# lmb-freiburg/understanding_flow_robustness

Measured on AMD Instinct MI355X. Metric: attack-iters/s, higher is better.
Workload: dtype f32

## Files before the change

include/ufr_hip.h:

```cpp
#ifndef UFR_HIP_H_
#define UFR_HIP_H_

#include <stdint.h>

#ifdef __cplusplus
extern "C" {
#endif

#define UFR_ABI_VERSION 9

enum { UFR_F32 = 0, UFR_F64 = 1, UFR_F16 = 2 };
enum {
  UFR_OK = 0,
  UFR_EINVAL = -1,
  UFR_EUNSUPPORTED = -2,
  UFR_ELAUNCH = -3
};

typedef void* ufr_stream_t;

int ufr_abi_version(void);
const char* ufr_last_error(void);
int ufr_device_count(void);
const char* ufr_build_manifest(void);
// ... 55 lines not shown
  float* grad_vol[UFR_MAX_LEVELS];
  int Hl[UFR_MAX_LEVELS], Wl[UFR_MAX_LEVELS];
} ufr_pyramid;

int ufr_corr_lookup_forward(const ufr_pyramid* pyr, const float* coords, float* out, int B, int H1,
                            int W1, int radius, ufr_stream_t stream);
int ufr_corr_lookup_backward(const ufr_pyramid* pyr, const float* coords, const float* grad_out,
                             int B, int H1, int W1, int radius, ufr_stream_t stream);

int ufr_resample2d_forward(const float* input1, const float* input2, float* output, int B, int C,
                           int Hi, int Wi, int H, int W, int kernel_size, int bilinear,
                           ufr_stream_t stream);
int ufr_resample2d_backward(const float* input1, const float* input2, const float* grad_output,
                            float* grad_input1, float* grad_input2, int B, int C, int Hi, int Wi,
                            int H, int W, int kernel_size, int bilinear, ufr_stream_t stream);
long ufr_resample2d_backward_workspace_bytes(int B, int H, int W);
int ufr_resample2d_backward_owner(const float* input1, const float* input2, const float* grad_output, float* grad_input1,
                                  float* grad_input2, void* workspace, long workspace_bytes, int B, int C, int H, int W,
                                  ufr_stream_t stream);

int ufr_flow_upscale4_forward(const float* flow, float* out, int B, int h, int w, int bilinear, float scale, int divide,
                              ufr_stream_t stream);
int ufr_flow_upscale4_backward(const float* grad_out, float* grad_flow, int B, int h, int w, int bilinear, float scale, int divide,
                               ufr_stream_t stream);
int ufr_fn2_stage_pack(const float* x, const float* resampled, const float* flow, float* out, int B, int H, int W, float div_flow,
                       ufr_stream_t stream);
int ufr_fn2_stage_unpack_grad(const float* grad_out, const float* packed, float* grad_x, float* grad_resampled, int B, int H, int W,
                              ufr_stream_t stream);
int ufr_fn2_stage_finish_grad(const float* grad_out, const float* grad_image, const float* grad_flow_rs, float* grad_x, float* grad_flow,
                              int B, int H, int W, float div_flow, ufr_stream_t stream);
int ufr_fn2_fusion_pack(const float* x, const float* flow_sd, const float* flow_s2, const float* res_sd, const float* res_s2, float* out,
                        int B, int H, int W, ufr_stream_t stream);
int ufr_fn2_fusion_unpack_grad(const float* grad_out, const float* packed, const float* res_sd, const float* res_s2, float* grad_x,
                               float* grad_res_sd, float* grad_res_s2, float* grad_flow_sd, float* grad_flow_s2, int B, int H, int W,
                               ufr_stream_t stream);
int ufr_fn2_fusion_finish_grad(const float* grad_image_sd, const float* grad_image_s2, const float* grad_flow_rs_sd,
                               const float* grad_flow_rs_s2, float* grad_x, float* grad_flow_sd, float* grad_flow_s2, int B, int H, int W,
                               ufr_stream_t stream);

int ufr_channelnorm_forward(const float* input1, float* output, int B, int C, int H, int W,
                            int norm_deg, ufr_stream_t stream);
int ufr_channelnorm_backward(const float* input1, const float* output, const float* grad_output,
                             float* grad_input1, int B, int C, int H, int W, int norm_deg,
                             ufr_stream_t stream);

int ufr_patch_paste(const float* tgt, const float* ref, const float* patch, const float* mask,
                    float* adv_tgt, float* adv_ref, int B, int CHW, long patch_bstride,
                    long mask_bstride, int do_clamp, float lo, float hi, ufr_stream_t stream);
int ufr_patch_update(const float* tgt, const float* ref, const float* g_tgt, const float* g_ref,
                     float* patch, const float* mask, float* adv_tgt, float* adv_ref, int B, int CHW,
                     long patch_bstride, long mask_bstride, float step, float bound, float lo, float hi,
                     const float* gate_state, ufr_stream_t stream);
int ufr_attack_gate(const float* loss_cur, float* state, float threshold, ufr_stream_t stream);
int ufr_patch_grad_crop(const float* g_tgt, const float* g_ref, const float* mask_p, const int* origins,
                        const int* origins_host, const float* loss_local, float* rows, int B, int H, int W,
                        int ph, int pw, int groups, ufr_stream_t stream);
int ufr_patch_grad_crop_window(const float* gxw, const int* win, const float* mask_p, const int* origins, const float* loss_local,
                               float* rows, int B, int H, int W, int wh, int ww, int ph, int pw, int groups, ufr_stream_t stream);
int ufr_patch_apply(const float* rows, int n_rows, float* patch_p, float* loss, int ph, int pw, float step,
                    float bound, const float* gate_state, ufr_stream_t stream);
int ufr_patch_paste_placed(const float* tgt, const float* ref, const float* patch_p, const float* mask_p,
                           const int* origins, const int* origins_host, float* adv_tgt, float* adv_ref,
                           float* mask_out, int B, int H, int W, int ph, int pw, int do_clamp, float lo, float hi,
                           const float* gate_state, ufr_stream_t stream);
int ufr_patch_paste_placed_rect(const float* tgt, const float* ref, const float* patch_p, const float* mask_p,
                                const int* origins, float* adv_tgt, float* adv_ref, int B, int H, int W, int ph, int pw,
                                int do_clamp, float lo, float hi, const float* gate_state, ufr_stream_t stream);
int ufr_attack_load_frames(const float* tgt, const float* ref, const float* patch_p, const float* mask_p, const int* origins,
                           float* tgt_dst, float* ref_dst, float* adv_tgt, float* adv_ref, int B, int H, int W, int ph, int pw,
                           ufr_stream_t stream);
int ufr_patch_mask_placed(const float* mask_p, const int* origins, float* mask_out, int B, int H, int W, int ph, int pw,
                          ufr_stream_t stream);
int ufr_patch_grad_crop_packed(const float* G, const int* win, const float* mask_p, const int* origins, const float* loss_local,
                               float* rows, int B, int H, int W, int wh, int ww, int ph, int pw, int groups, ufr_stream_t stream);
int ufr_patch_apply_paste_rect(const float* rows, int n_rows, float* patch_p, float* loss, const float* tgt, const float* ref,
                               const float* mask_p, const int* origins, float* adv_tgt, float* adv_ref, int B, int H, int W, int ph,
                               int pw, float step, float bound, int do_clamp, float lo, float hi, const float* gate_state,
                               ufr_stream_t stream);
#define UFR_LOSS_PARTIALS 1024
int ufr_flow_loss(const float* flow, const float* target, float* grad_flow, float* loss, int B,
                  int HW, int kind, float weight, float* partials, ufr_stream_t stream);
int ufr_flow2_upsampled_loss(const float* flow2, float flow_scale, const float* target, float* grad_flow2, float* loss, int B,
                             int h, int w, int kind, float weight, float* partials, ufr_stream_t stream);

int ufr_gru_gates_forward(const float* zr_pre, const float* h, float* z_out, float* rh_out, int B, int Ch,
                          int HW, long rh_bstride, ufr_stream_t stream);
int ufr_gru_gates_backward(const float* zr_pre, const float* h, const float* g_z, const float* g_rh,
                           float* g_zr, float* g_h, int B, int Ch, int HW, long grh_bstride,
                           ufr_stream_t stream);
int ufr_gru_blend_forward(const float* q_pre, const float* z, const float* h, float* h_out, long total,
                          ufr_stream_t stream);
int ufr_gru_blend_backward(const float* q_pre, const float* z, const float* h, const float* g, float* g_qpre,
                           float* g_z, float* g_h, long total, ufr_stream_t stream);

int ufr_raft_flow_patches(const float* flow, void* planes, long plane_stride, int chunk0, int B, int H, int W, ufr_stream_t stream);
int ufr_raft_motion_finish(void* p1, long plane_stride1, void* p2, long plane_stride2, int chunk0, const float* flow, int B, int H,
                           int W, ufr_stream_t stream);
int ufr_raft_motion_finish_slabs(const float* ws, int splitk, int Npad, int N, const float* bias, float slope, void* p1, long plane_stride1,
                                 void* p2, long plane_stride2, int chunk0, const float* flow, int B, int H, int W, ufr_stream_t stream);
int ufr_raft_coords_step(float* coords1, const float* delta, const float* coords0, float* saved, float* flow, long n, ufr_stream_t stream);
int ufr_grad_finalize_consume(float* g, const void* mask_plane0, void* out, long out_plane_stride, long M, int chunks, float slope,
                              ufr_stream_t stream);
int ufr_gru_gates_cm_forward(float* zr, const void* h, long h_plane_stride, int h_chunk0, void* rh, long rh_plane_stride,
                             int rh_chunk0, long M, int chunks, ufr_stream_t stream);
int ufr_gru_gates_cm_forward_slabs(const float* ws, int splitk, int Npad, const float* bias, const float* addend, float* zr, const void* h,
                                   long h_plane_stride, int h_chunk0, void* rh, long rh_plane_stride, int rh_chunk0, long M, int chunks,
                                   ufr_stream_t stream);
int ufr_gru_blend_cm_forward_slabs(const float* ws, int splitk, int Npad, const float* bias, const float* addend, float* q, const float* z,
                                   const void* h, long h_plane_stride, int h_chunk0, void* out, long out_plane_stride, int out_chunk0,
                                   long M, int chunks, ufr_stream_t stream);
int ufr_gru_blend_cm_forward(float* q, const float* z, const void* h, long h_plane_stride, int h_chunk0, void* out,
                             long out_plane_stride, int out_chunk0, long M, int chunks, ufr_stream_t stream);
int ufr_gru_blend_cm_backward(const float* q, const float* z, const void* h, long h_plane_stride, int h_chunk0, const float* g,
                              void* gq, long gq_plane_stride, int gq_chunk0, float* g_z, float* g_h, long M, int chunks,
                              float* acc_gq, ufr_stream_t stream);
int ufr_gru_gates_cm_backward(const float* zr, const void* h, long h_plane_stride, int h_chunk0, const float* g_z, float* g_rh,
                              void* gzr, long gzr_plane_stride, int gzr_chunk0, float* g_h, long M, int chunks, int consume_g_rh,
                              float* acc_gzr, ufr_stream_t stream);

long ufr_cm_norm_workspace_doubles(long HW, int n, int chunks);
int ufr_cm_norm_stats(const float* x, float* stats, double* workspace, long HW, int n, int chunks, float eps, ufr_stream_t stream);
int ufr_cm_norm_apply(const float* x, const float* stats, const void* res, long res_plane_stride, int res_chunk0, void* out,
                      long out_plane_stride, int out_chunk0, long HW, int n, int chunks, int relu1, int relu2, ufr_stream_t stream);
int ufr_cm_norm_stats_apply(const float* x, float* stats, double* workspace, float eps, const void* res, long res_plane_stride,
                            int res_chunk0, void* out, long out_plane_stride, int out_chunk0, long HW, int n, int chunks, int relu1,
                            int relu2, ufr_stream_t stream);
int ufr_cm_norm_backward(const float* x, const float* G, const void* outmask, int mask_chunk0, const float* stats, float* sums,
                         double* workspace, void* gz, long gz_plane_stride, int gz_chunk0, long HW, int n, int chunks, int relu1,
                         ufr_stream_t stream);
int ufr_cm_masked_copy(const float* G, const void* outmask, long mask_elem_offset, float* out, long elems, ufr_stream_t stream);

int ufr_conv3x3s2_c3_planes(const float* frames, const float* weight, const float* bias, float slope, void* out_planes,
                            long plane_stride, int out_chunk0, int n, int N, int H, int W, ufr_stream_t stream);

int ufr_conv3x3_c16_planes(const void* in_planes, long in_plane_stride, int in_chunk0, const float* weight_ct16, const float* bias,
                           float slope, void* out_planes, long out_plane_stride, int out_chunk0, int n, int H, int W, ufr_stream_t stream);

int ufr_pwc_warp_forward(const float* x, const float* flow, float* out, int B, int C, int H, int W,
                         ufr_stream_t stream);
int ufr_pwc_warp_backward(const float* x, const float* flow, const float* grad_out, float* grad_x, float* grad_flow,
                          int B, int C, int H, int W, ufr_stream_t stream);
long ufr_pwc_warp_backward_workspace_bytes(int B, int H, int W);
int ufr_pwc_warp_backward_owner(const float* x, const float* flow, const float* grad_out, float* grad_x, float* grad_flow,
                                void* workspace, long workspace_bytes, int B, int C, int H, int W, ufr_stream_t stream);

int ufr_raft_normalize_pair(const float* image1, const float* image2, float* stack, long n_each, ufr_stream_t stream);
int ufr_raft_normalize_pair_backward(const float* grad_stack, float* grad1, float* grad2, long n_each, ufr_stream_t stream);
int ufr_raft_fmap_pyramid_forward(const float* fmap, float* const* levels_nhwc, int levels, int B, int C, int H, int W,
                                  ufr_stream_t stream);
int ufr_raft_fmap_pyramid_backward(const float* const* grad_levels_nhwc, int levels, float* grad_fmap, int B, int C, int H, int W,
                                   ufr_stream_t stream);

int ufr_raft_context_split_forward(const float* ctx, float* net, float* inp, int B, int Ct, int Cr, long HW, ufr_stream_t stream);
int ufr_raft_context_split_backward(const float* net, const float* inp, const float* g_net, const float* g_inp, float* g_ctx,
                                    int B, int Ct, int Cr, long HW, ufr_stream_t stream);

int ufr_convex_upsample_forward(const float* flow, const float* mask, float* up, int N, int H, int W,
                                ufr_stream_t stream);
int ufr_convex_upsample_backward(const float* flow, const float* mask, const float* grad_up, float* grad_flow,
                                 float* grad_mask, float* workspace, int N, int H, int W, ufr_stream_t stream);

int ufr_flow_loss_ex(const float* flow, const float* gt, float* grad_flow, float* loss, int B, int HW,
                     int gt_channels, int kind, float scale, const float* scale_dev, float* partials,
                     ufr_stream_t stream);
int ufr_universal_update(const float* img0, const float* img1, const float* g0, const float* g1,
                         float* grad_sum, float* adv0, float* adv1, float* delta, int B, int CHW,
// ... 95 lines not shown
  int on;
  int row_tiles, col_tiles;
  int full_row_tiles, tail_row_tiles;
  int tail_row0, tail_rows;
  int slices, slice_ktiles, ktiles;
  int workgroups;
  long ws_floats;
  int steps_before, steps_after;
} ufr_igemm_tail_plan_t;
int ufr_igemm_tail_plan(const ufr_igemm_desc* d, int resident_workgroups, ufr_igemm_tail_plan_t* plan);
int ufr_igemm_balanced(const ufr_igemm_desc* d, int resident_workgroups, float* ws, long ws_floats, ufr_stream_t stream);
typedef struct {
  const void* x; long x_plane_stride; int in_chunk0, C;
  const void* gy; long gy_plane_stride; int g_chunk0, N;
  int B, Hi, Wi, Ho, Wo, kh, kw, sy, sx, py, px;
  float* dw;
  float* db;
  int accumulate;
  int splitm; float* ws; long ws_elems;
  int products;
} ufr_igemm_wgrad_desc;
int ufr_igemm_wgrad(const ufr_igemm_wgrad_desc* d, ufr_stream_t stream);
int ufr_igemm_wgrad_dilated(const ufr_igemm_wgrad_desc* d, int dy, int dx, ufr_stream_t stream);
int ufr_igemm_variant_fallbacks(void);
int ufr_igemm_clock_probe(unsigned long long* buf, int capacity_workgroups);
int ufr_rowmajor_to_planes(const float* src, long ld, long rows, int cols, float scale, void* planes, long plane_stride, int chunk0,
                           long plane_rows, ufr_stream_t stream);
int ufr_nchw_to_planes(const float* x, void* planes, long plane_stride, int chunk0, int B, int C, int H, int W,
                       float scale, float slope, const float* bias, ufr_stream_t stream);
int ufr_window_scatter_planes(const float* src, void* planes, long plane_stride, int chunk0, const int* win, int n_win,
                              int N, int C, int Hd, int Wd, int wh, int ww, int level_stride, int margin,
                              ufr_stream_t stream);
int ufr_window_features_planes(const void* c2w, long c2w_stride, const void* c3w, long c3w_stride, void* cat2, long cat2_stride,
                               void* c3a, long c3a_stride, void* c3b, long c3b_stride, float* c3_nchw, float* c3w_nchw,
                               const int* win, int B, int H, int W, int wh, int ww, int m2, int m3, ufr_stream_t stream);
int ufr_chunks_to_nchw(const void* planes, long plane_stride, const float* f32, int chunk0, const void* mask,
                       int mask_chunk0, float* out, int B, int C, int H, int W, float scale, float slope,
                       ufr_stream_t stream);
int ufr_nchw_cat_to_planes(const float* const* srcs, const int* channels, const int* dst_channel0, int nseg, void* planes,
                           long plane_stride, int chunk0, int chunks, int B, int H, int W, ufr_stream_t stream);
int ufr_chunks_to_nchw_cat(const float* g, int chunk0, int chunks, float* const* dsts, const int* channels, const int* src_channel0,
                           int nseg, const float* act0, float pos0, float neg0, int B, int H, int W, ufr_stream_t stream);
int ufr_grad_finalize(const float* g, int g_chunk0, const void* mask, int mask_chunk0, void* out, long out_plane_stride,
                      int out_chunk0, long M, int chunks, float slope, ufr_stream_t stream);

int ufr_conv1_direct(const float* frames_a, const float* frames_b, int Ba, int Bb, int H, int W, const double* mean,
                     const void* wimg, const float* bias, float slope, void* out_planes, long plane_stride, int out_chunk0,
                     ufr_stream_t stream);
int ufr_conv1_pack_planes(const float* frames_a, const float* frames_b, void* planes, long plane_stride, int Ba, int Bb, int H,
                          int W, const double* mean, ufr_stream_t stream);
int ufr_conv1_unpack_grad(const float* G, float* grad_frames, int N, int H, int W, ufr_stream_t stream);
int ufr_unshuffle_pack_planes(const float* x, void* planes, long plane_stride, int N, int C, int H, int W, ufr_stream_t stream);
int ufr_unshuffle_unpack_grad(const float* G, float* grad_x, int N, int C, int H, int W, ufr_stream_t stream);
int ufr_nchw_grad_to_planes(const float* grad, const float* act, void* planes, long plane_stride, int chunk0, int B, int C, int H,
                            int W, float slope, ufr_stream_t stream);
int ufr_window_gather_chunks(const float* src, float* dst, const int* win, int n_win, int N, int N_dst, int chunks, int Hs, int Ws,
                             int wh, int ww, int level_stride, int margin, ufr_stream_t stream);

int ufr_normalize_frames(const float* frames_a, const float* frames_b, float* out, int Ba, int Bb, int C, int H, int W,
                         const double* mean, ufr_stream_t stream);

int ufr_corr_forward_planes_window(const void* f1_planes, const void* f2_planes, long in_plane_stride, void* out_planes,
                                   long out_plane_stride, int out_chunk0, int B, int C, int H, int W, int patch,
                                   int dilation_patch, float scale, float slope, const int* win, int level_stride,
                                   int win_cells, ufr_stream_t stream);

int ufr_corr_forward_planes_changed(const void* f1_planes, const void* f2_planes, long in_plane_stride, void* out_planes,
                                    long out_plane_stride, int out_chunk0, int B, int C, int H, int W, int patch,
                                    int dilation_patch, float scale, float slope, const int* win, int level_stride,
                                    int win_cells_h, int win_cells_w, int margin, ufr_stream_t stream);

int ufr_corr_backward_window_fused(const float* f1, const float* f2, const float* G, int g_chunk0, float g_scale,
                                   const float* G_redir, float* grad_window, int B, int C, int H, int W, int patch,
                                   int dilation_patch, const int* win, int level_stride, int wh, int ww, int margin,
                                   ufr_stream_t stream);

int ufr_corr_forward_planes(const void* f1_planes, const void* f2_planes, long in_plane_stride, void* out_planes,
                            long out_plane_stride, int out_chunk0, int B, int C, int H, int W, int patch,
                            int dilation_patch, float scale, float slope, ufr_stream_t stream);
int ufr_flow_head_planes_forward(const void* planes, long plane_stride, int chunk0, int chunks, const float* wpk, int w_chunks,
                                 const float* bias, float* out, int B, int H, int W, ufr_stream_t stream);
int ufr_flow_head_planes_forward_mfma(const void* planes, long plane_stride, int chunk0, int chunks, const void* wmf, int w_chunks,
                                      const float* bias, float* out, int B, int H, int W, ufr_stream_t stream);
int ufr_deconv_flow_tail_backward_mfma(const void* grad_planes, long plane_stride, int chunk0, int chunks, const void* wmf,
                                       int w_chunks, float* G, int g_chunks, int out_chunk, int B, int H, int W, ufr_stream_t stream);
int ufr_flow_head_planes_backward(const float* grad_y, const float* wpk, int w_chunks, float* G, int g_chunks, int chunk0, int chunks,
                                  int B, int H, int W, int accumulate, ufr_stream_t stream);
int ufr_flow_head_planes_backward_finalize(const float* grad_y, const float* wpk, int w_chunks, float* G, int g_chunks, int chunk0,
                                           int chunks, int B, int H, int W, int accumulate, const void* mask_planes, void* out_planes,
                                           long out_plane_stride, int fin_chunk0, int fin_chunks, float slope, ufr_stream_t stream);
#define UFR_PF_REGION_BAND 1
#define UFR_PF_REGION_WINDOW 2
int ufr_flow_head_planes_backward_regions(const float* grad_y, const float* wpk, int w_chunks, float* G, int g_chunks, int chunk0,
                                          int chunks, int B, int H, int W, int accumulate, int head_chunks, int region,
                                          const int* origin, int origin_stride, int origin_div, int reg_h, int reg_w, int margin,
                                          float* head_out, int head_out_images, const void* mask_planes, void* out_planes,
                                          long out_plane_stride, int fin_chunk0, int fin_chunks, float slope, ufr_stream_t stream);
int ufr_upfeat_planes_forward_mfma(const void* planes, long plane_stride, int chunk0, int chunks, const void* wmf, int w_chunks,
                                   const float* bias, float* out, int B, int H, int W, ufr_stream_t stream);
int ufr_upfeat_planes_backward(const float* grad_y, const float* wpk, int w_chunks, float* G, int g_chunks, int chunk0, int chunks,
                               int B, int H, int W, int accumulate, ufr_stream_t stream);
int ufr_flow_up_planes_forward(const float* x, const float* w, const float* bias, void* planes, long plane_stride,
                               int chunk, int B, int H, int W, ufr_stream_t stream);
int ufr_flow_up_planes_backward(const float* G, int chunk, const float* w, float* grad_x, int B, int H, int W,
                                int accumulate , ufr_stream_t stream);

#define UFR_TRAIN_LOSS_MAX_SCALES 8
typedef struct {
  const float* gt; int B, H, W;
  int nscale;
  const float* pred[UFR_TRAIN_LOSS_MAX_SCALES];
  float* grad[UFR_TRAIN_LOSS_MAX_SCALES];
  int h[UFR_TRAIN_LOSS_MAX_SCALES], w[UFR_TRAIN_LOSS_MAX_SCALES];
  double weight[UFR_TRAIN_LOSS_MAX_SCALES];
  int kind;
  double div_flow;
  double* ws; long ws_elems;
  double* out;
} ufr_train_loss_desc;
long ufr_train_loss_workspace_doubles(int B, int nscale, const int* h, const int* w);
int ufr_train_loss(const ufr_train_loss_desc* d, ufr_stream_t stream);

typedef struct { float* p; const float* g; float* m; float* v; long n; } ufr_adamw_seg;
typedef struct { double lr, beta1, beta2, eps, weight_decay, bias1, bias2; } ufr_adamw_hyper;
long ufr_grad_norm_partials(const ufr_adamw_seg* segs, int nseg);
int ufr_grad_norm(const ufr_adamw_seg* segs, int nseg, float max_norm, double* partials, long partial_elems, float* norm_out,
                  ufr_stream_t stream);
int ufr_adamw_step(const ufr_adamw_seg* segs, int nseg, const ufr_adamw_hyper* h, const float* norm, ufr_stream_t stream);

int ufr_sweep_paste(const float* tgt, const float* ref, const float* patch_p, const float* mask_p, const int* origins,
                    const int* origins_host, float* adv_tgt, float* adv_ref, int K, int H, int W, int ph, int pw, float lo, float hi,
                    const ufr_cone_chain* chain, int win_h, int win_w, int* win, float* xw, ufr_stream_t stream);
long ufr_sweep_metrics_workspace_doubles(int K);
int ufr_sweep_metrics(const float* pred, const float* gt, const float* mask_p, const int* origins, const int* origins_host, int K,
                      int H, int W, int Hg, int Wg, int ph, int pw, int valid_in_patch, double* ws, long ws_elems, float* out,
                      int row0, int rows, ufr_stream_t stream);

#define UFR_FEATURE_STATS_MAX_SEGS 32
typedef struct {
  const void* src; long plane_stride; long pixels; int kind, images, image0, B, chunk0, channels; double unleaky; long out_col;
} ufr_feature_stats_seg;
long ufr_feature_stats_workspace_doubles(const ufr_feature_stats_seg* segs, int nseg);
int ufr_feature_stats(const ufr_feature_stats_seg* segs, int nseg, double* ws, long ws_elems, double* out, int out_rows, long out_cols,
                      long out_stride, ufr_stream_t stream);

#define UFR_DIVERSE_COLS 8
long ufr_abs_sums_workspace_doubles(long n);
int ufr_abs_sums(const float* g0, const float* g1, long n, double* ws, long ws_elems, float* out, ufr_stream_t stream);
int ufr_momentum_update(const float* img0, const float* img1, const float* g0, const float* g1, const float* sums, float* m0,
                        float* m1, float* adv0, float* adv1, float* delta, int B, int CHW, float mu, float one_minus_mu, float lr,
                        float eps, float lo, float hi, int frames, int ascent, ufr_stream_t stream);
int ufr_diverse_table_check(const int* table_host, int rows, int H, int W);
long ufr_diverse_workspace_doubles(int B, int H, int W, int Cg);
int ufr_diverse_forward(const float* adv0, const float* adv1, const float* gt, float* x0, float* x1, float* gt_out, int B, int H,
                        int W, int Cg, const int* table, int rows, const int* step, float* scale_t, double* ws, long ws_elems,
                        ufr_stream_t stream);
int ufr_diverse_backward(const float* gx0, const float* gx1, float* g0, float* g1, int B, int H, int W, const int* table, int rows,
                         const int* step, ufr_stream_t stream);
int ufr_step_advance(int* step, ufr_stream_t stream);

#ifdef __cplusplus
}
#endif
#endif
```

understanding_flow_robustness_amd/_lib.py:

```python
from __future__ import annotations

import ctypes as C
import os

import torch

_HERE = os.path.dirname(os.path.abspath(__file__))
LIB_PATH = os.environ.get("UFR_HIP_LIB") or os.path.join(_HERE, "lib", "libufr_hip.so")
UFR_F32, UFR_F64, UFR_F16 = 0, 1, 2
ABI_VERSION = 9
_lib = None


class CorrParams(C.Structure):
    _fields_ = [(n, C.c_int) for n in (
        "kH", "kW", "patchH", "patchW", "padH", "padW", "dilationH", "dilationW",
        "dilation_patchH", "dilation_patchW", "dH", "dW")]


UFR_MAX_LEVELS = 8


class Pyramid(C.Structure):
    _fields_ = [("num_levels", C.c_int),
# ... 49 lines not shown
                ("tail_row0", C.c_int), ("tail_rows", C.c_int), ("slices", C.c_int), ("slice_ktiles", C.c_int), ("ktiles", C.c_int),
                ("workgroups", C.c_int), ("ws_floats", C.c_long), ("steps_before", C.c_int), ("steps_after", C.c_int)]


UFR_IGEMM_WGRAD_MAX_TAPS = 49


class IgemmWgradDesc(C.Structure):
    _fields_ = [("x", C.c_void_p), ("x_plane_stride", C.c_long), ("in_chunk0", C.c_int), ("C", C.c_int),
                ("gy", C.c_void_p), ("gy_plane_stride", C.c_long), ("g_chunk0", C.c_int), ("N", C.c_int),
                ("B", C.c_int), ("Hi", C.c_int), ("Wi", C.c_int), ("Ho", C.c_int), ("Wo", C.c_int),
                ("kh", C.c_int), ("kw", C.c_int), ("sy", C.c_int), ("sx", C.c_int), ("py", C.c_int), ("px", C.c_int),
                ("dw", C.c_void_p), ("db", C.c_void_p), ("accumulate", C.c_int),
                ("splitm", C.c_int), ("ws", C.c_void_p), ("ws_elems", C.c_long),
                ("products", C.c_int)]


UFR_TRAIN_LOSS_MAX_SCALES = 8


class TrainLossDesc(C.Structure):
    _fields_ = [("gt", C.c_void_p), ("B", C.c_int), ("H", C.c_int), ("W", C.c_int), ("nscale", C.c_int),
                ("pred", C.c_void_p * UFR_TRAIN_LOSS_MAX_SCALES), ("grad", C.c_void_p * UFR_TRAIN_LOSS_MAX_SCALES),
                ("h", C.c_int * UFR_TRAIN_LOSS_MAX_SCALES), ("w", C.c_int * UFR_TRAIN_LOSS_MAX_SCALES),
                ("weight", C.c_double * UFR_TRAIN_LOSS_MAX_SCALES),
                ("kind", C.c_int), ("div_flow", C.c_double),
                ("ws", C.c_void_p), ("ws_elems", C.c_long), ("out", C.c_void_p)]


class AdamwSeg(C.Structure):
    _fields_ = [("p", C.c_void_p), ("g", C.c_void_p), ("m", C.c_void_p), ("v", C.c_void_p), ("n", C.c_long)]


class AdamwHyper(C.Structure):
    _fields_ = [(n, C.c_double) for n in ("lr", "beta1", "beta2", "eps", "weight_decay", "bias1", "bias2")]


class FeatureStatsSeg(C.Structure):
    _fields_ = [("src", C.c_void_p), ("plane_stride", C.c_long), ("pixels", C.c_long), ("kind", C.c_int), ("images", C.c_int),
                ("image0", C.c_int), ("B", C.c_int), ("chunk0", C.c_int), ("channels", C.c_int), ("unleaky", C.c_double),
                ("out_col", C.c_long)]


UFR_FEATURE_STATS_MAX_SEGS = 32
UFR_MAX_CONE_LAYERS = 8
UFR_PF_REGION_BAND, UFR_PF_REGION_WINDOW = 1, 2


class ConeChain(C.Structure):
    _fields_ = [("n_layers", C.c_int),
                ("kernel", C.c_int * UFR_MAX_CONE_LAYERS), ("stride", C.c_int * UFR_MAX_CONE_LAYERS),
                ("pad", C.c_int * UFR_MAX_CONE_LAYERS),
                ("n_taps", C.c_int),
                ("tap_layer", C.c_int * UFR_MAX_CONE_LAYERS), ("tap_margin", C.c_int * UFR_MAX_CONE_LAYERS)]


_vp, _i, _f, _l, _d = C.c_void_p, C.c_int, C.c_float, C.c_long, C.c_double
LOSS_PARTIALS = 1024
SIGNATURES = {
    "ufr_corr_forward": [_vp, _vp, _vp, _i, _i, _i, _i, _i, C.POINTER(CorrParams), _vp],
    "ufr_corr_forward_fused": [_vp, _vp, _vp, _i, _i, _i, _i, _i, C.POINTER(CorrParams), _f, _f, _vp],
    "ufr_corr_backward": [_vp, _vp, _vp, _vp, _vp, _i, _i, _i, _i, _i, C.POINTER(CorrParams), _vp],
    "ufr_altcorr_forward": [_vp, _vp, _vp, _vp, _i, _i, _i, _i, _i, _i, _i, _i, _vp],
    "ufr_altcorr_backward": [_vp, _vp, _vp, _vp, _vp, _vp, _vp, _i, _i, _i, _i, _i, _i, _i, _i, _vp],
    "ufr_corr_lookup_forward": [C.POINTER(Pyramid), _vp, _vp, _i, _i, _i, _i, _vp],
    "ufr_corr_lookup_backward": [C.POINTER(Pyramid), _vp, _vp, _i, _i, _i, _i, _vp],
    "ufr_resample2d_forward": [_vp, _vp, _vp, _i, _i, _i, _i, _i, _i, _i, _i, _vp],
    "ufr_resample2d_backward_owner": [_vp, _vp, _vp, _vp, _vp, _vp, _l, _i, _i, _i, _i, _vp],
    "ufr_resample2d_backward": [_vp, _vp, _vp, _vp, _vp, _i, _i, _i, _i, _i, _i, _i, _i, _vp],
    "ufr_channelnorm_forward": [_vp, _vp, _i, _i, _i, _i, _i, _vp],
    "ufr_channelnorm_backward": [_vp, _vp, _vp, _vp, _i, _i, _i, _i, _i, _vp],
    "ufr_patch_paste": [_vp, _vp, _vp, _vp, _vp, _vp, _i, _i, _l, _l, _i, _f, _f, _vp],
    "ufr_patch_update": [_vp, _vp, _vp, _vp, _vp, _vp, _vp, _vp, _i, _i, _l, _l, _f, _f, _f, _f, _vp, _vp],
    "ufr_attack_gate": [_vp, _vp, _f, _vp],
    "ufr_gru_gates_forward": [_vp, _vp, _vp, _vp, _i, _i, _i, _l, _vp],
    "ufr_gru_gates_backward": [_vp, _vp, _vp, _vp, _vp, _vp, _i, _i, _i, _l, _vp],
    "ufr_gru_blend_forward": [_vp, _vp, _vp, _vp, _l, _vp],
    "ufr_gru_blend_backward": [_vp, _vp, _vp, _vp, _vp, _vp, _vp, _l, _vp],
    "ufr_flow_loss_ex": [_vp, _vp, _vp, _vp, _i, _i, _i, _i, _f, _vp, _vp, _vp],
    "ufr_universal_update": [_vp, _vp, _vp, _vp, _vp, _vp, _vp, _vp, _i, _i, _f, _f, _f, _f, _i, _i, _i, _i,
                             _i, _vp],
    "ufr_flow_loss": [_vp, _vp, _vp, _vp, _i, _i, _i, _f, _vp, _vp],
    "ufr_flow2_upsampled_loss": [_vp, _f, _vp, _vp, _vp, _i, _i, _i, _i, _f, _vp, _vp],
    "ufr_patch_grad_crop": [_vp, _vp, _vp, _vp, _vp, _vp, _vp, _i, _i, _i, _i, _i, _i, _vp],
    "ufr_patch_apply": [_vp, _i, _vp, _vp, _i, _i, _f, _f, _vp, _vp],
    "ufr_patch_grad_crop_window": [_vp, _vp, _vp, _vp, _vp, _vp, _i, _i, _i, _i, _i, _i, _i, _i, _vp],
    "ufr_patch_paste_placed_rect": [_vp, _vp, _vp, _vp, _vp, _vp, _vp, _i, _i, _i, _i, _i, _i, _f, _f, _vp, _vp],
    "ufr_patch_paste_placed": [_vp, _vp, _vp, _vp, _vp, _vp, _vp, _vp, _vp, _i, _i, _i, _i, _i, _i, _f, _f, _vp, _vp],
    "ufr_cone_window": [_vp, _i, _l, _i, _i, _i, C.POINTER(ConeChain), _i, _i, _vp, _vp, _vp],
    "ufr_attack_place": [_vp, _vp, _vp, _vp, _vp, _vp, _vp, _vp, _vp, _vp, _vp, _i, _i, _i, _i, _i, C.POINTER(ConeChain), _i, _i,
                         _vp, _vp, _i, _i, _i, _i, _vp],
    "ufr_attack_load_frames": [_vp, _vp, _vp, _vp, _vp, _vp, _vp, _vp, _vp, _i, _i, _i, _i, _i, _vp],
    "ufr_patch_mask_placed": [_vp, _vp, _vp, _i, _i, _i, _i, _i, _vp],
    "ufr_patch_grad_crop_packed": [_vp, _vp, _vp, _vp, _vp, _vp, _i, _i, _i, _i, _i, _i, _i, _i, _vp],
    "ufr_patch_apply_paste_rect": [_vp, _i, _vp, _vp, _vp, _vp, _vp, _vp, _vp, _vp, _i, _i, _i, _i, _i, _f, _f, _i, _f, _f, _vp, _vp],
    "ufr_window_gather_pair": [_vp, _vp, _vp, _vp, _vp, _i, _i, _i, _i, _i, _i, _vp],
    "ufr_window_features_planes": [_vp, _l, _vp, _l, _vp, _l, _vp, _l, _vp, _l, _vp, _vp, _vp, _i, _i, _i, _i, _i, _i, _i, _vp],
    "ufr_window_gather": [_vp, _vp, _vp, _i, _i, _i, _i, _i, _i, _i, _i, _i, _vp],
    "ufr_window_scatter": [_vp, _vp, _vp, _i, _i, _i, _i, _i, _i, _i, _i, _i, _vp],
    "ufr_conv1_pack_planes": [_vp, _vp, _vp, _l, _i, _i, _i, _i, _vp, _vp],
    "ufr_conv1_unpack_grad": [_vp, _vp, _i, _i, _i, _vp],
    "ufr_nchw_grad_to_planes": [_vp, _vp, _vp, _l, _i, _i, _i, _i, _i, _f, _vp],
    "ufr_window_gather_chunks": [_vp, _vp, _vp, _i, _i, _i, _i, _i, _i, _i, _i, _i, _i, _vp],
    "ufr_normalize_frames": [_vp, _vp, _vp, _i, _i, _i, _i, _i, _vp, _vp],
    "ufr_corr_backward_window_fused": [_vp, _vp, _vp, _i, _f, _vp, _vp, _i, _i, _i, _i, _i, _i, _vp, _i, _i, _i, _i, _vp],
    "ufr_corr_backward_window": [_vp, _vp, _vp, _vp, _vp, _i, _i, _i, _i, _i, _i, _vp, _i, _i, _i, _vp],
    "ufr_bias_leaky_forward": [_vp, _vp, _i, _i, _l, _f, _vp],
    "ufr_leaky_backward": [_vp, _vp, _vp, _l, _f, _vp],
    "ufr_conv3x3_c2_forward": [_vp, _vp, _vp, _vp, _vp, _i, _i, _i, _i, _vp],
    "ufr_conv3x3_c2_backward_data": [_vp, _vp, _vp, _i, _i, _i, _i, _vp],
    "ufr_deconv4x4s2_c2_forward": [_vp, _vp, _vp, _vp, _i, _i, _i, _vp],
    "ufr_deconv4x4s2_c2_backward_data": [_vp, _vp, _vp, _i, _i, _i, _vp],
    "ufr_pwc_warp_forward": [_vp, _vp, _vp, _i, _i, _i, _i, _vp],
    "ufr_pwc_warp_backward": [_vp, _vp, _vp, _vp, _vp, _i, _i, _i, _i, _vp],
    "ufr_pwc_warp_backward_owner": [_vp, _vp, _vp, _vp, _vp, _vp, _l, _i, _i, _i, _i, _vp],
    "ufr_raft_normalize_pair": [_vp, _vp, _vp, _l, _vp],
    "ufr_raft_normalize_pair_backward": [_vp, _vp, _vp, _l, _vp],
    "ufr_raft_fmap_pyramid_forward": [_vp, _vp, _i, _i, _i, _i, _i, _vp],
    "ufr_raft_fmap_pyramid_backward": [_vp, _i, _vp, _i, _i, _i, _i, _vp],
    "ufr_raft_context_split_forward": [_vp, _vp, _vp, _i, _i, _i, _l, _vp],
    "ufr_raft_context_split_backward": [_vp, _vp, _vp, _vp, _vp, _i, _i, _i, _l, _vp],
    "ufr_igemm": [C.POINTER(IgemmDesc), _vp],
    "ufr_igemm_tail_plan": [C.POINTER(IgemmDesc), _i, C.POINTER(IgemmTailPlan)],
    "ufr_igemm_balanced": [C.POINTER(IgemmDesc), _i, _vp, _l, _vp],
    "ufr_igemm_wgrad": [C.POINTER(IgemmWgradDesc), _vp],
    "ufr_igemm_wgrad_dilated": [C.POINTER(IgemmWgradDesc), _i, _i, _vp],
    "ufr_flow_upscale4_forward": [_vp, _vp, _i, _i, _i, _i, _f, _i, _vp],
    "ufr_flow_upscale4_backward": [_vp, _vp, _i, _i, _i, _i, _f, _i, _vp],
    "ufr_fn2_stage_pack": [_vp, _vp, _vp, _vp, _i, _i, _i, _f, _vp],
    "ufr_fn2_stage_unpack_grad": [_vp, _vp, _vp, _vp, _i, _i, _i, _vp],
    "ufr_fn2_stage_finish_grad": [_vp, _vp, _vp, _vp, _vp, _i, _i, _i, _f, _vp],
    "ufr_fn2_fusion_pack": [_vp, _vp, _vp, _vp, _vp, _vp, _i, _i, _i, _vp],
    "ufr_fn2_fusion_unpack_grad": [_vp, _vp, _vp, _vp, _vp, _vp, _vp, _vp, _vp, _i, _i, _i, _vp],
    "ufr_fn2_fusion_finish_grad": [_vp, _vp, _vp, _vp, _vp, _vp, _vp, _i, _i, _i, _vp],
    "ufr_rowmajor_to_planes": [_vp, _l, _l, _i, _f, _vp, _l, _i, _l, _vp],
    "ufr_nchw_to_planes": [_vp, _vp, _l, _i, _i, _i, _i, _i, _f, _f, _vp, _vp],
    "ufr_window_scatter_planes": [_vp, _vp, _l, _i, _vp, _i, _i, _i, _i, _i, _i, _i, _i, _i, _vp],
    "ufr_chunks_to_nchw": [_vp, _l, _vp, _i, _vp, _i, _vp, _i, _i, _i, _i, _f, _f, _vp],
    "ufr_nchw_cat_to_planes": [_vp, _vp, _vp, _i, _vp, _l, _i, _i, _i, _i, _i, _vp],
    "ufr_chunks_to_nchw_cat": [_vp, _i, _i, _vp, _vp, _vp, _i, _vp, _f, _f, _i, _i, _i, _vp],
    "ufr_grad_finalize": [_vp, _i, _vp, _i, _vp, _l, _i, _l, _i, _f, _vp],
    "ufr_flow_head_planes_forward": [_vp, _l, _i, _i, _vp, _i, _vp, _vp, _i, _i, _i, _vp],
    "ufr_flow_head_planes_forward_mfma": [_vp, _l, _i, _i, _vp, _i, _vp, _vp, _i, _i, _i, _vp],
    "ufr_deconv_flow_tail_backward_mfma": [_vp, _l, _i, _i, _vp, _i, _vp, _i, _i, _i, _i, _i, _vp],
    "ufr_flow_head_planes_backward": [_vp, _vp, _i, _vp, _i, _i, _i, _i, _i, _i, _i, _vp],
    "ufr_flow_head_planes_backward_finalize": [_vp, _vp, _i, _vp, _i, _i, _i, _i, _i, _i, _i, _vp, _vp, _l, _i, _i, _f, _vp],
    "ufr_flow_head_planes_backward_regions": [_vp, _vp, _i, _vp, _i, _i, _i, _i, _i, _i, _i, _i, _i, _vp, _i, _i, _i, _i, _i, _vp, _i,
                                              _vp, _vp, _l, _i, _i, _f, _vp],
    "ufr_unshuffle_pack_planes": [_vp, _vp, _l, _i, _i, _i, _i, _vp],
    "ufr_unshuffle_unpack_grad": [_vp, _vp, _i, _i, _i, _i, _vp],
    "ufr_conv3x3s2_c3_planes": [_vp, _vp, _vp, _f, _vp, _l, _i, _i, _i, _i, _i, _vp],
    "ufr_conv3x3_c16_planes": [_vp, _l, _i, _vp, _vp, _f, _vp, _l, _i, _i, _i, _i, _vp],
    "ufr_cm_norm_stats": [_vp, _vp, _vp, _l, _i, _i, _f, _vp],
    "ufr_cm_norm_apply": [_vp, _vp, _vp, _l, _i, _vp, _l, _i, _l, _i, _i, _i, _i, _vp],
    "ufr_cm_norm_stats_apply": [_vp, _vp, _vp, _f, _vp, _l, _i, _vp, _l, _i, _l, _i, _i, _i, _i, _vp],
    "ufr_cm_norm_backward": [_vp, _vp, _vp, _i, _vp, _vp, _vp, _vp, _l, _i, _l, _i, _i, _i, _vp],
    "ufr_cm_masked_copy": [_vp, _vp, _l, _vp, _l, _vp],
    "ufr_raft_flow_patches": [_vp, _vp, _l, _i, _i, _i, _i, _vp],
    "ufr_raft_motion_finish_slabs": [_vp, _i, _i, _i, _vp, _f, _vp, _l, _vp, _l, _i, _vp, _i, _i, _i, _vp],
    "ufr_raft_motion_finish": [_vp, _l, _vp, _l, _i, _vp, _i, _i, _i, _vp],
    "ufr_raft_coords_step": [_vp, _vp, _vp, _vp, _vp, _l, _vp],
    "ufr_grad_finalize_consume": [_vp, _vp, _vp, _l, _l, _i, _f, _vp],
    "ufr_gru_gates_cm_forward": [_vp, _vp, _l, _i, _vp, _l, _i, _l, _i, _vp],
    "ufr_gru_gates_cm_forward_slabs": [_vp, _i, _i, _vp, _vp, _vp, _vp, _l, _i, _vp, _l, _i, _l, _i, _vp],
    "ufr_gru_blend_cm_forward_slabs": [_vp, _i, _i, _vp, _vp, _vp, _vp, _vp, _l, _i, _vp, _l, _i, _l, _i, _vp],
    "ufr_gru_blend_cm_forward": [_vp, _vp, _vp, _l, _i, _vp, _l, _i, _l, _i, _vp],
    "ufr_gru_blend_cm_backward": [_vp, _vp, _vp, _l, _i, _vp, _vp, _l, _i, _vp, _vp, _l, _i, _vp, _vp],
    "ufr_gru_gates_cm_backward": [_vp, _vp, _l, _i, _vp, _vp, _vp, _l, _i, _vp, _l, _i, _i, _vp, _vp],
    "ufr_altcorr_pyramid_forward": [_vp, _vp, _vp, _vp, _i, _i, _i, _i, _i, _f, _vp],
    "ufr_altcorr_pyramid_backward": [_vp, _vp, _vp, _vp, _vp, _vp, _i, _i, _i, _i, _i, _f, _i, _vp],
    "ufr_altcorr_pyramid_backward_cm": [_vp, _vp, _vp, _vp, _vp, _vp, _i, _i, _i, _i, _i, _f, _i, _vp],
    "ufr_upfeat_planes_forward_mfma": [_vp, _l, _i, _i, _vp, _i, _vp, _vp, _i, _i, _i, _vp],
    "ufr_upfeat_planes_backward": [_vp, _vp, _i, _vp, _i, _i, _i, _i, _i, _i, _i, _vp],
    "ufr_flow_up_planes_forward": [_vp, _vp, _vp, _vp, _l, _i, _i, _i, _i, _vp],
    "ufr_flow_up_planes_backward": [_vp, _i, _vp, _vp, _i, _i, _i, _i, _vp],
    "ufr_corr_forward_planes_changed": [_vp, _vp, _l, _vp, _l, _i, _i, _i, _i, _i, _i, _i, _f, _f, _vp, _i, _i, _i, _i, _vp],
    "ufr_corr_forward_planes_window": [_vp, _vp, _l, _vp, _l, _i, _i, _i, _i, _i, _i, _i, _f, _f, _vp, _i, _i, _vp],
    "ufr_corr_forward_planes": [_vp, _vp, _l, _vp, _l, _i, _i, _i, _i, _i, _i, _i, _f, _f, _vp],
    "ufr_convex_upsample_forward": [_vp, _vp, _vp, _i, _i, _i, _vp],
    "ufr_convex_upsample_backward": [_vp, _vp, _vp, _vp, _vp, _vp, _i, _i, _i, _vp],
    "ufr_affine_resample_f64": [_vp, _vp, _i, _i, _i, _i, _i, _d, _d, _d, _d, _d, _d, _i, _vp],
    "ufr_patch_place": [_vp, _vp, _vp, _i, _i, _i, _vp, _vp, _vp, _i, _i, _i, _i, _vp],
    "ufr_patch_crop_f64": [_vp, _vp, _vp, _i, _i, _i, _i, _i, _i, _i, _vp],
    "ufr_resample_u8_horizontal": [_vp, _vp, _i, _i, _i, _i, _i, _vp, _vp, _i, _vp],
    "ufr_resample_u8_vertical": [_vp, _vp, _i, _i, _i, _i, _vp, _vp, _i, _vp],
    "ufr_u8_to_tensor": [_vp, _vp, _i, _i, _i, _i, _i, _i, _i, _f, _vp],
    "ufr_kitti_flow_decode": [_vp, _vp, _i, _i, _vp],
    "ufr_host_png_unfilter": [_vp, _vp, _i, _i, _i],
    "ufr_igemm_clock_probe": [_vp, _i],
    "ufr_altcorr_planes_prepare": [_vp, _vp, _l, _l, _i, _vp],
    "ufr_altcorr_planes_forward": [_vp, _l, C.POINTER(AltCorrPlaneLevels), _vp, _vp, _i, _i, _i, _i, _i, _f, _vp],
    "ufr_conv1_direct": [_vp, _vp, _i, _i, _i, _i, _vp, _vp, _vp, _f, _vp, _l, _i, _vp],
    "ufr_train_loss": [C.POINTER(TrainLossDesc), _vp],
    "ufr_grad_norm": [C.POINTER(AdamwSeg), _i, _f, _vp, _l, _vp, _vp],
    "ufr_adamw_step": [C.POINTER(AdamwSeg), _i, C.POINTER(AdamwHyper), _vp, _vp],
    "ufr_sweep_paste": [_vp, _vp, _vp, _vp, _vp, _vp, _vp, _vp, _i, _i, _i, _i, _i, _f, _f, C.POINTER(ConeChain), _i, _i, _vp, _vp, _vp],
    "ufr_sweep_metrics": [_vp, _vp, _vp, _vp, _vp, _i, _i, _i, _i, _i, _i, _i, _i, _vp, _l, _vp, _i, _i, _vp],
    "ufr_feature_stats": [C.POINTER(FeatureStatsSeg), _i, _vp, _l, _vp, _i, _l, _l, _vp],
    "ufr_abs_sums": [_vp, _vp, _l, _vp, _l, _vp, _vp],
    "ufr_momentum_update": [_vp, _vp, _vp, _vp, _vp, _vp, _vp, _vp, _vp, _vp, _i, _i, _f, _f, _f, _f, _f, _f, _i, _i, _vp],
    "ufr_diverse_table_check": [_vp, _i, _i, _i],
    "ufr_diverse_forward": [_vp, _vp, _vp, _vp, _vp, _vp, _i, _i, _i, _i, _vp, _i, _vp, _vp, _vp, _l, _vp],
    "ufr_diverse_backward": [_vp, _vp, _vp, _vp, _i, _i, _i, _vp, _i, _vp, _vp],
    "ufr_step_advance": [_vp, _vp],
}
DIVERSE_COLS = 8
PLAIN = {"ufr_abi_version": (C.c_int, []), "ufr_last_error": (C.c_char_p, []),
         "ufr_device_count": (C.c_int, []), "ufr_build_manifest": (C.c_char_p, []),
         "ufr_igemm_variant_fallbacks": (C.c_int, []),
         "ufr_conv3x3_c2_workspace_floats": (C.c_long, [_i, _i, _i, _i]),
         "ufr_cm_norm_workspace_doubles": (C.c_long, [_l, _i, _i]),
         "ufr_resample2d_backward_workspace_bytes": (C.c_long, [_i, _i, _i]),
         "ufr_pwc_warp_backward_workspace_bytes": (C.c_long, [_i, _i, _i]),
         "ufr_altcorr_pyramid_workspace_bytes": (C.c_long, [_i, _i, _i, _i, _i, _i]),
         "ufr_train_loss_workspace_doubles": (C.c_long, [_i, _i, C.POINTER(C.c_int), C.POINTER(C.c_int)]),
         "ufr_grad_norm_partials": (C.c_long, [C.POINTER(AdamwSeg), _i]),
         "ufr_sweep_metrics_workspace_doubles": (C.c_long, [_i]),
         "ufr_feature_stats_workspace_doubles": (C.c_long, [C.POINTER(FeatureStatsSeg), _i]),
         "ufr_abs_sums_workspace_doubles": (C.c_long, [_l]),
         "ufr_diverse_workspace_doubles": (C.c_long, [_i, _i, _i, _i])}


def lib():
    global _lib
    if _lib is None:
        if not os.path.exists(LIB_PATH):
            raise RuntimeError(
                f"{LIB_PATH} not found: build it with `python -c 'import __graft_entry__ as g; "
                "g.build()'` or `make -C understanding_flow_robustness_amd/csrc` (hipcc, gfx950). "
                "There is no CPU fallback.")
        handle = C.CDLL(LIB_PATH)
        for name, args in SIGNATURES.items():
            fn = getattr(handle, name)
            fn.argtypes, fn.restype = args, C.c_int
        for name, (res, args) in PLAIN.items():
            fn = getattr(handle, name)
            fn.argtypes, fn.restype = args, res
        if handle.ufr_abi_version() != ABI_VERSION:
            raise RuntimeError(f"{LIB_PATH} has ABI version {handle.ufr_abi_version()}, these bindings are written for "
                               f"{ABI_VERSION}: rebuild it (`make -C understanding_flow_robustness_amd/csrc`)")
        verify_build(handle.ufr_build_manifest().decode("ascii", "replace"))
        _lib = handle
    return _lib


_CSRC = os.path.join(_HERE, "csrc")
_HEADER = os.path.join(os.path.dirname(_HERE), "include", "ufr_hip.h")


def source_checksums(csrc: str = _CSRC, header: str = _HEADER) -> dict:
    import hashlib
    with open(os.path.join(csrc, "ufr_common.h"), "rb") as f:
        shared = f.read()
    with open(header, "rb") as f:
        shared += f.read()
    sums = {}
    for name in sorted(os.listdir(csrc)):
# ... 226 lines not shown
```

understanding_flow_robustness_amd/csrc/attack.hip:

```cpp
#include "ufr_common.h"

namespace {

__device__ __forceinline__ float clampf(float v, float lo, float hi) { return fminf(fmaxf(v, lo), hi); }

__global__ void paste_kernel(const float* __restrict__ tgt, const float* __restrict__ ref,
                             const float* __restrict__ patch, const float* __restrict__ mask,
                             float* __restrict__ adv_tgt, float* __restrict__ adv_ref, long total,
                             long CHW, long pstride, long mstride, int do_clamp, float lo, float hi) {
  for (long i = (long)blockIdx.x * blockDim.x + threadIdx.x; i < total;
       i += (long)gridDim.x * blockDim.x) {
    const long b = i / CHW, e = i - b * CHW;
    const float m = mask[b * mstride + e], pv = patch[b * pstride + e];
    const float mp = m * pv, om = 1.0f - m;
    float a = om * tgt[i] + mp;
    float r = om * ref[i] + mp;
    if (do_clamp) { a = clampf(a, lo, hi); r = clampf(r, lo, hi); }
    adv_tgt[i] = a;
    adv_ref[i] = r;
  }
}

__global__ void update_private_kernel(const float* __restrict__ tgt, const float* __restrict__ ref,
                                      const float* __restrict__ g_tgt, const float* __restrict__ g_ref,
// ... 423 lines not shown
      const float fu = hy0 * (wx0 * f2[0][a0][c0] + lx * f2[0][a0][c1]) + ly * (wx0 * f2[0][a1][c0] + lx * f2[0][a1][c1]);
      const float fv = hy0 * (wx0 * f2[1][a0][c0] + lx * f2[1][a0][c1]) + ly * (wx0 * f2[1][a1][c0] + lx * f2[1][a1][c1]);
      const long o0 = ((long)b * 2) * HW + (long)py * W + px, o1 = o0 + HW;
      const float tu = target[o0], tv = target[o1];
      float term;
      if (kind == 0) {
        const float dot = fu * tu + fv * tv;
        const float nf2 = fu * fu + fv * fv, nt2 = tu * tu + tv * tv;
        const float den = fmaxf(sqrtf(nf2 * nt2), 1e-8f);
        const float c = dot / den;
        term = 1.0f - c;
        if (sqrtf(nf2 * nt2) > 1e-8f) {
          gu = -(tu / den - c * fu / nf2);
          gv = -(tv / den - c * fv / nf2);
        } else {
          gu = -(tu / den);
          gv = -(tv / den);
        }
      } else {
        const float du = fu - tu, dv = fv - tv;
        const float sd = sqrtf(du * du + dv * dv + 1e-8f);
        term = sd;
        gu = du / sd;
        gv = dv / sd;
      }
      gu *= invn;
      gv *= invn;
      const bool owned = ry >= 4 && ry < F2_R - 4 && rx >= 4 && rx < F2_R - 4;
      if (owned) part += term;
    }
    g[0][ry][rx] = gu;
    g[1][ry][rx] = gv;
  }
  __syncthreads();
  {
    const int cyl = tid >> 4, cxl = tid & 15, cy = cy0 + cyl, cx = cx0 + cxl;
    if (cy < h && cx < w) {
      float su = 0.f, sv = 0.f;
      for (int py = 4 * cy - 3; py <= 4 * cy + 6; ++py) {
        if (py < 0 || py >= H) continue;
        int y0, y1;
        float ly;
        up4_source(py, h, y0, y1, ly);
        const float wy = (y0 == cy ? 1.f - ly : 0.f) + (y1 == cy ? ly : 0.f);
        if (wy == 0.f) continue;
        float ru = 0.f, rv = 0.f;
        for (int px = 4 * cx - 3; px <= 4 * cx + 6; ++px) {
          if (px < 0 || px >= W) continue;
          int x0, x1;
          float lx;
          up4_source(px, w, x0, x1, lx);
          const float wx = (x0 == cx ? 1.f - lx : 0.f) + (x1 == cx ? lx : 0.f);
          ru += wx * g[0][py - py0][px - px0];
          rv += wx * g[1][py - py0][px - px0];
        }
        su += wy * ru;
        sv += wy * rv;
      }
      gflow2[((long)b * 2) * hw + (long)cy * w + cx] = su * flow_scale;
      gflow2[((long)b * 2 + 1) * hw + (long)cy * w + cx] = sv * flow_scale;
    }
  }
  for (int off = 32; off > 0; off >>= 1) part += __shfl_down(part, off, 64);
  if ((tid & 63) == 0) red[tid >> 6] = part;
  __syncthreads();
  if (tid == 0) partials[(blockIdx.z * gridDim.y + blockIdx.y) * gridDim.x + blockIdx.x] = (red[0] + red[1] + red[2] + red[3]) * invn;
}

extern "C" int ufr_flow2_upsampled_loss(const float* flow2, float flow_scale, const float* target, float* grad_flow2, float* loss,
                                        int B, int h, int w, int kind, float weight, float* partials, ufr_stream_t stream) {
  UFR_REQUIRE(flow2 && target && grad_flow2 && loss && partials, "upsampled flow loss: null pointer argument");
  UFR_REQUIRE(B > 0 && h > 0 && w > 0 && (kind == 0 || kind == 1), "upsampled flow loss: bad argument");
  const dim3 grid(ufr::ceil_div(w, F2_T), ufr::ceil_div(h, F2_T), B);
  const long n = (long)grid.x * grid.y * grid.z;
  if (n > UFR_LOSS_PARTIALS || B > 65535)
    return ufr::fail(UFR_EUNSUPPORTED, "upsampled flow loss: %ld tiles exceed the %d partial sums of the fixed-order reduction", n,
                     UFR_LOSS_PARTIALS);
  hipLaunchKernelGGL(flow2_upsampled_loss_kernel, grid, dim3(256), 0, ufr::as_stream(stream), flow2, flow_scale, target, grad_flow2,
                     partials, B, h, w, kind, weight);
  hipLaunchKernelGGL(loss_finalize_kernel, dim3(1), dim3(64), 0, ufr::as_stream(stream), partials, (int)n, loss);
  return ufr::launched("flow2_upsampled_loss_kernel");
}

namespace ufr {
void loss_finalize_launch(const float* partials, int n, float* loss, hipStream_t st) {
  hipLaunchKernelGGL(loss_finalize_kernel, dim3(1), dim3(64), 0, st, partials, n, loss);
}
}

static int check_placed(const int* origins_host, int B, int H, int W, int ph, int pw) {
  if (!origins_host) return 1;
  for (int b = 0; b < B; ++b)
    if (origins_host[2 * b] < 0 || origins_host[2 * b] + ph > H || origins_host[2 * b + 1] < 0 ||
        origins_host[2 * b + 1] + pw > W)
      return 0;
  return 1;
}

extern "C" int ufr_patch_grad_crop(const float* g_tgt, const float* g_ref, const float* mask_p, const int* origins,
                                   const int* origins_host, const float* loss_local, float* rows, int B, int H, int W,
                                   int ph, int pw, int groups, ufr_stream_t stream) {
  UFR_REQUIRE(g_tgt && g_ref && mask_p && origins && loss_local && rows, "patch grad crop: null pointer argument");
  UFR_REQUIRE(B > 0 && H > 0 && W > 0 && ph > 0 && pw > 0 && ph <= H && pw <= W, "patch grad crop: bad shape");
  UFR_REQUIRE(groups > 0 && B % groups == 0, "patch grad crop: the pairs must split evenly into %d groups", groups);
  UFR_REQUIRE(check_placed(origins_host, B, H, W, ph, pw), "patch grad crop: a placement leaves the frame");
  const int n = 3 * ph * pw + 1;
  hipLaunchKernelGGL(patch_grad_crop_kernel, dim3(ufr::ceil_div(n, 256)), dim3(256), 0, ufr::as_stream(stream), g_tgt,
                     g_ref, mask_p, origins, loss_local, rows, B, H, W, ph, pw, groups);
  return ufr::launched("patch_grad_crop_kernel");
}

extern "C" int ufr_patch_grad_crop_window(const float* gxw, const int* win, const float* mask_p, const int* origins,
                                          const float* loss_local, float* rows, int B, int H, int W, int wh, int ww, int ph, int pw,
                                          int groups, ufr_stream_t stream) {
  UFR_REQUIRE(gxw && win && mask_p && origins && loss_local && rows, "patch grad crop (window): null pointer argument");
  UFR_REQUIRE(B > 0 && H > 0 && W > 0 && ph > 0 && pw > 0 && ph <= H && pw <= W && wh > 0 && ww > 0 && wh <= H && ww <= W,
              "patch grad crop (window): bad shape");
  UFR_REQUIRE(groups > 0 && B % groups == 0, "patch grad crop (window): the pairs must split evenly into %d groups", groups);
  const int n = 3 * ph * pw + 1;
  hipLaunchKernelGGL(patch_grad_crop_window_kernel, dim3(ufr::ceil_div(n, 256)), dim3(256), 0, ufr::as_stream(stream), gxw, win,
                     mask_p, origins, loss_local, rows, B, H, W, wh, ww, ph, pw, groups);
  return ufr::launched("patch_grad_crop_window_kernel");
}

extern "C" int ufr_patch_apply(const float* rows, int n_rows, float* patch_p, float* loss, int ph, int pw, float step,
                               float bound, const float* gate_state, ufr_stream_t stream) {
  UFR_REQUIRE(rows && patch_p && loss, "patch apply: null pointer argument");
  UFR_REQUIRE(n_rows > 0 && ph > 0 && pw > 0, "patch apply: bad shape");
  const int n = 3 * ph * pw;
  hipLaunchKernelGGL(patch_apply_kernel, dim3(ufr::ceil_div(n + 1, 256)), dim3(256), 0, ufr::as_stream(stream), rows,
                     n_rows, patch_p, loss, n, step, bound, gate_state);
  return ufr::launched("patch_apply_kernel");
}

extern "C" int ufr_patch_paste_placed(const float* tgt, const float* ref, const float* patch_p, const float* mask_p,
                                      const int* origins, const int* origins_host, float* adv_tgt, float* adv_ref,
                                      float* mask_out, int B, int H, int W, int ph, int pw, int do_clamp, float lo,
                                      float hi, const float* gate_state, ufr_stream_t stream) {
  UFR_REQUIRE(tgt && ref && patch_p && mask_p && origins && adv_tgt && adv_ref, "placed paste: null pointer argument");
  UFR_REQUIRE(B > 0 && H > 0 && W > 0 && ph > 0 && pw > 0 && ph <= H && pw <= W, "placed paste: bad shape");
  UFR_REQUIRE(check_placed(origins_host, B, H, W, ph, pw), "placed paste: a placement leaves the frame");
  const long total = (long)B * 3 * H * W;
  hipLaunchKernelGGL(paste_placed_kernel, dim3(ufr::stream_grid(total, 256)), dim3(256), 0, ufr::as_stream(stream), tgt,
                     ref, patch_p, mask_p, origins, adv_tgt, adv_ref, mask_out, total, H, W, ph, pw, do_clamp, lo, hi,
                     gate_state);
  return ufr::launched("paste_placed_kernel");
}

extern "C" int ufr_patch_paste_placed_rect(const float* tgt, const float* ref, const float* patch_p, const float* mask_p,
                                           const int* origins, float* adv_tgt, float* adv_ref, int B, int H, int W, int ph, int pw,
                                           int do_clamp, float lo, float hi, const float* gate_state, ufr_stream_t stream) {
  UFR_REQUIRE(tgt && ref && patch_p && mask_p && origins && adv_tgt && adv_ref, "placed rect paste: null pointer argument");
  UFR_REQUIRE(B > 0 && H > 0 && W > 0 && ph > 0 && pw > 0 && ph <= H && pw <= W, "placed rect paste: bad shape");
  const long total = (long)B * 3 * ph * pw;
  UFR_REQUIRE(total < (1L << 30), "placed rect paste: too many patch pixels");
  hipLaunchKernelGGL(paste_placed_rect_kernel, dim3(ufr::stream_grid(total, 256)), dim3(256), 0, ufr::as_stream(stream), tgt, ref,
                     patch_p, mask_p, origins, adv_tgt, adv_ref, B, H, W, ph, pw, do_clamp, lo, hi, gate_state);
  return ufr::launched("paste_placed_rect_kernel");
}

extern "C" int ufr_attack_load_frames(const float* tgt, const float* ref, const float* patch_p, const float* mask_p,
                                      const int* origins, float* tgt_dst, float* ref_dst, float* adv_tgt, float* adv_ref, int B,
                                      int H, int W, int ph, int pw, ufr_stream_t stream) {
  UFR_REQUIRE(tgt && ref && patch_p && mask_p && origins && tgt_dst && ref_dst && adv_tgt && adv_ref,
              "attack load frames: null pointer argument");
  UFR_REQUIRE(B > 0 && H > 0 && W > 0 && ph > 0 && pw > 0 && ph <= H && pw <= W, "attack load frames: bad shape");
// ... 60 lines not shown
```

understanding_flow_robustness_amd/csrc/engine_small.hip:

```cpp
#include "ufr_common.h"

namespace {

typedef __attribute__((ext_vector_type(8))) __bf16 bf16x8;

__device__ __forceinline__ void split3(float v, __bf16& a, __bf16& b, __bf16& c) {
  a = (__bf16)v;
  const float r1 = v - (float)a;
  b = (__bf16)r1;
  c = (__bf16)(r1 - (float)b);
}

constexpr int PF_TH = 8, PF_TW = 32, PF_HH = PF_TH + 2, PF_HW = PF_TW + 2, PF_CS = 36;
__global__ __launch_bounds__(1024) void flow_head_planes_fwd(const __bf16* __restrict__ x, long plane_stride, int chunk0,
                                                             int chunks, const float* __restrict__ wpk,
                                                             const float* __restrict__ bias, float* __restrict__ out, int B,
                                                             int H, int W, int S) {
  extern __shared__ __attribute__((aligned(16))) float lds_pf[];
  const long M = (long)B * H * W;
  const int tid = threadIdx.x, slice = tid >> 8, t = tid & 255;
  float* tile = lds_pf + (long)slice * (PF_HH * PF_HW * PF_CS);
  float* part = lds_pf + (long)S * (PF_HH * PF_HW * PF_CS + 576);
  const int tiles_x = (W + PF_TW - 1) / PF_TW, tiles_y = (H + PF_TH - 1) / PF_TH;
  const int b = blockIdx.x / (tiles_x * tiles_y), tr = blockIdx.x - b * tiles_x * tiles_y;
// ... 185 lines not shown
#pragma unroll
      for (int s = 0; s < 6; ++s)
        if (tw + WPS_ * (h + s) < mt) {
#pragma unroll
          for (int nt = 0; nt < 2; ++nt)
#pragma unroll
            for (int q = 0; q < 6; ++q)
              acc[h + s][nt] = __builtin_amdgcn_mfma_f32_16x16x32_bf16(fa[s][PFM_A[q]], fb[nt][PFM_B[q]], acc[h + s][nt], 0, 0, 0);
        }
    }
  }
  float* T = pfm_T + (long)slice * mt * 16 * TS;
#pragma unroll
  for (int s = 0; s < MAXT_; ++s)
    if (tw + WPS_ * s < mt) {
#pragma unroll
      for (int r = 0; r < 4; ++r) {
        float* row = T + ((tw + WPS_ * s) * 16 + (lane >> 4) * 4 + r) * TS;
        row[lane & 15] = acc[s][0][r];
        if (MODE != 0 || (lane & 15) < 2) row[16 + (lane & 15)] = acc[s][1][r];
      }
    }
  __syncthreads();
  if constexpr (MODE == 2) {
    const int Ho = 2 * H, Wo = 2 * W;
    for (int idx = tid; idx < 2 * TH * 32; idx += blockDim.x) {
      const int ly = idx >> 5, lx = idx & 31;
      const int Y = 2 * y0 + ly, X = 2 * x0 + lx;
      if (Y >= Ho || X >= Wo) continue;
      float r0 = 0.f, r1 = 0.f;
      for (int sl = 0; sl < S; ++sl) {
        const float* Ts = pfm_T + (long)sl * mt * 16 * TS;
#pragma unroll
        for (int t = 0; t < 2; ++t) {
          const int ky = ((Y + 1) & 1) + 2 * t, hy = (Y + 1 - ky) / 2 - sy0;
#pragma unroll
          for (int u = 0; u < 2; ++u) {
            const int kx = ((X + 1) & 1) + 2 * u, hx = (X + 1 - kx) / 2 - sx0;
            const float* e = Ts + (hy * PFM_HW + hx) * TS + 2 * (ky * 4 + kx);
            r0 += e[0];
            r1 += e[1];
          }
        }
      }
      const long HWo = (long)Ho * Wo, p = (long)Y * Wo + X;
      out[((long)b * 2 + 0) * HWo + p] = r0 + bias[0];
      out[((long)b * 2 + 1) * HWo + p] = r1 + bias[1];
    }
    return;
  }
  if (tid < TH * TW) {
    const int ly = tid / TW, lx = tid - ly * TW;
    const int yy = y0 + ly, xx = x0 + lx;
    if (yy < H && xx < W) {
      float r0 = 0.f, r1 = 0.f;
      for (int sl = 0; sl < S; ++sl) {
        const float* Ts = pfm_T + (long)sl * mt * 16 * TS;
        if (MODE == 0) {
#pragma unroll
          for (int k = 0; k < 9; ++k) {
            const float* e = Ts + ((ly + k / 3) * PFM_HW + lx + k % 3) * TS + 2 * k;
            r0 += e[0];
            r1 += e[1];
          }
        } else {
#pragma unroll
          for (int k = 0; k < 16; ++k) {
            const float* e = Ts + ((2 * ly + k / 4) * PFM_HW + 2 * lx + k % 4) * TS + 2 * k;
            r0 += e[0];
            r1 += e[1];
          }
        }
      }
      if (MODE == 0) {
        const long HW = (long)H * W, p = (long)yy * W + xx;
        out[((long)b * 2 + 0) * HW + p] = r0 + bias[0];
        out[((long)b * 2 + 1) * HW + p] = r1 + bias[1];
      } else {
        float* o = out + ((long)out_chunk * B * H * W + ((long)b * H + yy) * W + xx) * 32;
        o[0] = r0;
        o[1] = r1;
      }
    }
  }
}

struct PfFinalize {
  const __bf16* mask; __bf16* out; long out_plane_stride; int c0, n; float slope;
};

__device__ __forceinline__ void pf_bwd_taps(const float* __restrict__ gy, long b, int yy, int xx, int H, int W, float (&g0)[9],
                                            float (&g1)[9]) {
  const long HW = (long)H * W;
#pragma unroll
  for (int k = 0; k < 9; ++k) {
    const int y2 = yy - (k / 3 - 1), x2 = xx - (k % 3 - 1);
    const bool ok = y2 >= 0 && y2 < H && x2 >= 0 && x2 < W;
    g0[k] = ok ? gy[(b * 2 + 0) * HW + (long)y2 * W + x2] : 0.f;
    g1[k] = ok ? gy[(b * 2 + 1) * HW + (long)y2 * W + x2] : 0.f;
  }
}

__device__ __forceinline__ void pf_bwd_chunk(const float* wc, const float (&g0)[9], const float (&g1)[9], float4& lo, float4& hi) {
  float a[8] = {0.f, 0.f, 0.f, 0.f, 0.f, 0.f, 0.f, 0.f};
#pragma unroll
  for (int k = 0; k < 9; ++k) {
    const float4 w0a = *reinterpret_cast<const float4*>(wc + (k * 2 + 0) * 32), w0b = *reinterpret_cast<const float4*>(wc + (k * 2 + 0) * 32 + 4);
    const float w0[8] = {w0a.x, w0a.y, w0a.z, w0a.w, w0b.x, w0b.y, w0b.z, w0b.w};
#pragma unroll
    for (int j = 0; j < 8; ++j) a[j] = fmaf(g0[k], w0[j], a[j]);
  }
#pragma unroll
  for (int k = 0; k < 9; ++k) {
    const float4 w1a = *reinterpret_cast<const float4*>(wc + (k * 2 + 1) * 32), w1b = *reinterpret_cast<const float4*>(wc + (k * 2 + 1) * 32 + 4);
    const float w1[8] = {w1a.x, w1a.y, w1a.z, w1a.w, w1b.x, w1b.y, w1b.z, w1b.w};
#pragma unroll
    for (int j = 0; j < 8; ++j) a[j] = fmaf(g1[k], w1[j], a[j]);
  }
  lo = make_float4(a[0], a[1], a[2], a[3]);
  hi = make_float4(a[4], a[5], a[6], a[7]);
}

__device__ __forceinline__ void pf_bwd_store(float* p, int accumulate, float4& lo, float4& hi) {
  float4* dst = reinterpret_cast<float4*>(p);
  if (accumulate) {
    const float4 o0 = dst[0], o1 = dst[1];
    lo.x += o0.x; lo.y += o0.y; lo.z += o0.z; lo.w += o0.w;
    hi.x += o1.x; hi.y += o1.y; hi.z += o1.z; hi.w += o1.w;
  }
  dst[0] = lo;
  dst[1] = hi;
}

__device__ __forceinline__ void pf_bwd_finalize(const PfFinalize& fin, long e, const float4& lo, const float4& hi) {
  float v[8] = {lo.x, lo.y, lo.z, lo.w, hi.x, hi.y, hi.z, hi.w};
  if (fin.mask) {
    const bf16x8 m = *reinterpret_cast<const bf16x8*>(fin.mask + e);
#pragma unroll
    for (int j = 0; j < 8; ++j) v[j] = ((float)m[j] > 0.f) ? v[j] : v[j] * fin.slope;
  }
  bf16x8 q0, q1, q2;
#pragma unroll
  for (int j = 0; j < 8; ++j) {
    __bf16 x, y, z;
    split3(v[j], x, y, z);
    q0[j] = x; q1[j] = y; q2[j] = z;
  }
  *reinterpret_cast<bf16x8*>(fin.out + e) = q0;
  *reinterpret_cast<bf16x8*>(fin.out + e + fin.out_plane_stride) = q1;
  *reinterpret_cast<bf16x8*>(fin.out + e + 2 * fin.out_plane_stride) = q2;
}

__global__ __launch_bounds__(256) void flow_head_planes_bwd(const float* __restrict__ gy, const float* __restrict__ wpk,
                                                            float* __restrict__ G, int chunk0, int chunks, int B, int H, int W,
                                                            int accumulate, int per, const PfFinalize fin) {
  extern __shared__ __attribute__((aligned(16))) float lds_w[];
  const long M = (long)B * H * W;
  const int c_lo = blockIdx.y * per, c_hi = min(chunks, c_lo + per);
  for (int i = threadIdx.x; i < (c_hi - c_lo) * 576 / 4; i += blockDim.x)
    reinterpret_cast<float4*>(lds_w)[i] = reinterpret_cast<const float4*>(wpk + (long)c_lo * 576)[i];
  __syncthreads();
  const long t = (long)blockIdx.x * blockDim.x + threadIdx.x;
  const long pix = t >> 2;
  const int q = (int)(t & 3);
  if (pix >= M) return;
  const long HW = (long)H * W, b = pix / HW, p = pix - b * HW;
// ... 175 lines not shown
      o[0] = v; o[1] = zero; o[2] = zero; o[3] = zero;
    }
  }
}

__global__ void flow_up_planes_bwd(const float* __restrict__ G, int chunk, const float* __restrict__ w, float* __restrict__ gx,
                                   int B, int H, int W, int accumulate) {
  const int Ho = 2 * H, Wo = 2 * W;
  const long total = (long)B * H * W, Mf = (long)B * Ho * Wo;
  for (long i = (long)blockIdx.x * blockDim.x + threadIdx.x; i < total; i += (long)gridDim.x * blockDim.x) {
    const int xx = (int)(i % W), yy = (int)((i / W) % H), b = (int)(i / ((long)W * H));
    float a0 = 0.f, a1 = 0.f;
#pragma unroll
    for (int ky = 0; ky < 4; ++ky) {
      const int Y = 2 * yy - 1 + ky;
      if (Y < 0 || Y >= Ho) continue;
#pragma unroll
      for (int kx = 0; kx < 4; ++kx) {
        const int X = 2 * xx - 1 + kx;
        if (X < 0 || X >= Wo) continue;
        const float2 g = *reinterpret_cast<const float2*>(G + ((long)chunk * Mf + ((long)b * Ho + Y) * Wo + X) * 32);
        a0 = fmaf(g.x, w[((0 * 2 + 0) * 4 + ky) * 4 + kx], a0);
        a1 = fmaf(g.x, w[((1 * 2 + 0) * 4 + ky) * 4 + kx], a1);
        a0 = fmaf(g.y, w[((0 * 2 + 1) * 4 + ky) * 4 + kx], a0);
        a1 = fmaf(g.y, w[((1 * 2 + 1) * 4 + ky) * 4 + kx], a1);
      }
    }
    float* o0 = gx + ((size_t)b * 2 + 0) * H * W + (size_t)yy * W + xx;
    float* o1 = gx + ((size_t)b * 2 + 1) * H * W + (size_t)yy * W + xx;
    *o0 = accumulate ? *o0 + a0 : a0;
    *o1 = accumulate ? *o1 + a1 : a1;
  }
}

bool planes_hold(long plane_stride, long pixels, int chunk0, int chunks) {
  return plane_stride > 0 && (long)(chunk0 + chunks) * pixels * 32 <= plane_stride;
}
#define UFR_REQUIRE_RANGE(what, plane_stride, pixels, chunk0, chunks, w_chunks)                                                       \
  do {                                                                                                                                \
    if (!planes_hold(plane_stride, pixels, chunk0, chunks))                                                                           \
      return ufr::fail(UFR_EINVAL, "%s: chunks [%d, %d) leave the planes operand (%ld chunks per plane)", what, chunk0,               \
                       chunk0 + chunks, (long)(plane_stride) / ((long)(pixels) * 32));                                               \
    if ((chunks) > (w_chunks))                                                                                                        \
      return ufr::fail(UFR_EINVAL, "%s: %d chunks asked of packed weights that hold %d", what, chunks, w_chunks);                     \
  } while (0)
#define UFR_REQUIRE_GRANGE(what, chunk0, chunks, w_chunks, g_chunks)                                                                  \
  do {                                                                                                                                \
    if ((chunk0) + (chunks) > (g_chunks))                                                                                             \
      return ufr::fail(UFR_EINVAL, "%s: chunks [%d, %d) leave the gradient sum (%d chunks)", what, chunk0, chunk0 + chunks, g_chunks); \
    if ((chunks) > (w_chunks))                                                                                                        \
      return ufr::fail(UFR_EINVAL, "%s: %d chunks asked of packed weights that hold %d", what, chunks, w_chunks);                     \
  } while (0)

}

extern "C" int ufr_flow_head_planes_forward(const void* planes, long plane_stride, int chunk0, int chunks, const float* wpk, int w_chunks,
                                            const float* bias, float* out, int B, int H, int W, ufr_stream_t stream) {
  UFR_REQUIRE(planes && wpk && bias && out, "flow head (planes) forward: null pointer");
  UFR_REQUIRE(B > 0 && H > 0 && W > 0 && chunks > 0 && chunks <= 48 && chunk0 >= 0 && (long)B * H * W < (1L << 29),
              "flow head (planes) forward: bad shape");
  UFR_REQUIRE_RANGE("flow head (planes) forward", plane_stride, (long)B * H * W, chunk0, chunks, w_chunks);
  const int blocks = B * ufr::ceil_div(H, PF_TH) * ufr::ceil_div(W, PF_TW);
  hipStream_t st = ufr::as_stream(stream);
  (void)ufr::ensure_dynamic_lds(reinterpret_cast<const void*>(flow_head_planes_fwd), (2 * (PF_HH * PF_HW * PF_CS + 576) + 2 * 256 * 2) * 4);
  (void)ufr::ensure_dynamic_lds(reinterpret_cast<const void*>(flow_head_planes_fwd_small), 48 * 576 * 4 + 4 * 64 * 2 * 4);
  if (blocks >= 192) {
    const int S = (blocks < 512 && chunks >= 8) ? 2 : 1;
    const size_t lds = ((size_t)S * (PF_HH * PF_HW * PF_CS + 576) + (size_t)S * 256 * 2) * 4;
    flow_head_planes_fwd<<<blocks, 256 * S, lds, st>>>(static_cast<const __bf16*>(planes), plane_stride, chunk0, chunks, wpk, bias,
                                                       out, B, H, W, S);
    return ufr::launched("flow_head_planes_fwd");
  }
  const long M = (long)B * H * W;
  const int sblocks = ufr::ceil_div(M, 64);
  int S = 1;
  while (S < 4 && (long)sblocks * S * 2 <= 2048 && chunks >= 4 * S) S *= 2;
  const size_t lds = (size_t)chunks * 576 * 4 + (size_t)S * 64 * 2 * 4;
  flow_head_planes_fwd_small<<<sblocks, 256 * S, lds, st>>>(static_cast<const __bf16*>(planes), plane_stride, chunk0, chunks, wpk,
                                                           bias, out, B, H, W, S);
  return ufr::launched("flow_head_planes_fwd_small");
}

namespace {
template <int MODE>
int launch_pf_mfma(const void* planes, long plane_stride, int chunk0, int chunks, const void* wmf, const float* bias, float* out,
                   int out_chunk, int B, int H, int W, hipStream_t st, const char* what) {
  constexpr int TW = MODE == 0 ? 32 : 16, TS = MODE == 0 ? 20 : 36, HWs = MODE == 2 ? 18 : 34;
  auto blocks_of = [&](int th) { return B * ufr::ceil_div(H, th) * ufr::ceil_div(W, TW); };
  int TH;
  if (MODE == 0) TH = blocks_of(8) >= 512 ? 8 : (blocks_of(4) >= 256 ? 4 : 2);
  else if (MODE == 1) TH = blocks_of(4) >= 256 ? 4 : 2;
  else TH = blocks_of(16) >= 512 ? 16 : (blocks_of(8) >= 256 ? 8 : 4);
  const int blocks = blocks_of(TH);
  const int S = (blocks >= 512 || chunks < 4) ? 1 : 2;
  const int mt = ((MODE == 1 ? 2 * TH + 2 : TH + 2) * HWs + 15) / 16;
  const size_t lds = (size_t)S * mt * 16 * TS * sizeof(float);
  if (lds > 64 * 1024) {
    hipError_t e = ufr::ensure_dynamic_lds(reinterpret_cast<const void*>(flow_head_planes_fwd_mfma<MODE>), lds);
    if (e != hipSuccess) return ufr::fail(UFR_ELAUNCH, "%s: %s", what, hipGetErrorString(e));
  }
  if constexpr (MODE == 0) if (mt <= 12 && S == 2 && chunks >= 16 && blocks <= 256) {
    const size_t lds8 = (size_t)8 * mt * 16 * TS * sizeof(float);
    hipError_t e = ufr::ensure_dynamic_lds(reinterpret_cast<const void*>(flow_head_planes_fwd_mfma<MODE, 1, 12>),
                                           8 * 12 * 16 * TS * sizeof(float));
    if (e != hipSuccess) return ufr::fail(UFR_ELAUNCH, "%s: %s", what, hipGetErrorString(e));
    flow_head_planes_fwd_mfma<MODE, 1, 12><<<blocks, 512, lds8, st>>>(static_cast<const __bf16*>(planes), plane_stride, chunk0, chunks,
                                                                      static_cast<const __bf16*>(wmf), bias, out, out_chunk, B, H, W, TH, 8);
    return ufr::launched(what);
  }
  flow_head_planes_fwd_mfma<MODE><<<blocks, 256 * S, lds, st>>>(static_cast<const __bf16*>(planes), plane_stride, chunk0, chunks,
                                                                static_cast<const __bf16*>(wmf), bias, out, out_chunk, B, H, W, TH, S);
  return ufr::launched(what);
}
}

extern "C" int ufr_flow_head_planes_forward_mfma(const void* planes, long plane_stride, int chunk0, int chunks, const void* wmf,
                                                 int w_chunks, const float* bias, float* out, int B, int H, int W, ufr_stream_t stream) {
  UFR_REQUIRE(planes && wmf && bias && out, "flow head (planes, mfma) forward: null pointer");
  UFR_REQUIRE(B > 0 && H > 0 && W > 0 && chunks > 0 && chunks <= 48 && chunk0 >= 0 && (long)B * H * W < (1L << 29),
              "flow head (planes, mfma) forward: bad shape");
  UFR_REQUIRE_RANGE("flow head (planes, mfma) forward", plane_stride, (long)B * H * W, chunk0, chunks, w_chunks);
  return launch_pf_mfma<0>(planes, plane_stride, chunk0, chunks, wmf, bias, out, 0, B, H, W, ufr::as_stream(stream),
                           "flow_head_planes_fwd_mfma");
}

extern "C" int ufr_deconv_flow_tail_backward_mfma(const void* grad_planes, long plane_stride, int chunk0, int chunks, const void* wmf,
                                                  int w_chunks, float* G, int g_chunks, int out_chunk, int B, int H, int W,
                                                  ufr_stream_t stream) {
  UFR_REQUIRE(grad_planes && wmf && G, "deconv flow tail backward: null pointer");
  UFR_REQUIRE(B > 0 && H > 0 && W > 0 && chunks > 0 && chunks <= 48 && chunk0 >= 0 && out_chunk >= 0 &&
                  (long)B * H * W < (1L << 27), "deconv flow tail backward: bad shape");
  UFR_REQUIRE_RANGE("deconv flow tail backward", plane_stride, (long)B * H * W * 4, chunk0, chunks, w_chunks);
  UFR_REQUIRE(out_chunk < g_chunks, "deconv flow tail backward: chunk %d is not in the gradient sum (%d chunks)", out_chunk, g_chunks);
  return launch_pf_mfma<1>(grad_planes, plane_stride, chunk0, chunks, wmf, nullptr, G, out_chunk, B, H, W, ufr::as_stream(stream),
                           "deconv_flow_tail_bwd_mfma");
}

extern "C" int ufr_upfeat_planes_forward_mfma(const void* planes, long plane_stride, int chunk0, int chunks, const void* wmf,
                                              int w_chunks, const float* bias, float* out, int B, int H, int W, ufr_stream_t stream) {
  UFR_REQUIRE(planes && wmf && bias && out, "upfeat (planes, mfma) forward: null pointer");
  UFR_REQUIRE(B > 0 && H > 0 && W > 0 && chunks > 0 && chunks <= 48 && chunk0 >= 0 && (long)B * H * W < (1L << 27),
              "upfeat (planes, mfma) forward: bad shape");
  UFR_REQUIRE_RANGE("upfeat (planes, mfma) forward", plane_stride, (long)B * H * W, chunk0, chunks, w_chunks);
  return launch_pf_mfma<2>(planes, plane_stride, chunk0, chunks, wmf, bias, out, 0, B, H, W, ufr::as_stream(stream),
                           "upfeat_planes_fwd_mfma");
}

extern "C" int ufr_upfeat_planes_backward(const float* grad_y, const float* wpk, int w_chunks, float* G, int g_chunks, int chunk0,
                                          int chunks, int B, int H, int W, int accumulate, ufr_stream_t stream) {
  UFR_REQUIRE(grad_y && wpk && G, "upfeat (planes) backward: null pointer");
  UFR_REQUIRE(B > 0 && H > 0 && W > 0 && chunks > 0 && chunks <= 48 && chunk0 >= 0 && (long)B * H * W < (1L << 27),
              "upfeat (planes) backward: bad shape");
  UFR_REQUIRE_GRANGE("upfeat (planes) backward", chunk0, chunks, w_chunks, g_chunks);
  const long threads = (long)B * H * W * 4;
  const int bx = ufr::ceil_div(threads, 256);
  int slices = 1;
  while ((long)bx * slices < 1024 && slices < chunks) slices *= 2;
  if (slices > chunks) slices = chunks;
  int per = ufr::ceil_div(chunks, slices);
  if (per > 12) per = 12;
  slices = ufr::ceil_div(chunks, per);
  flow_tail_planes_bwd<<<dim3(bx, slices), 256, (size_t)per * 1024 * 4, ufr::as_stream(stream)>>>(grad_y, wpk, G, chunk0, chunks, B,
                                                                                                 H, W, accumulate, per);
  return ufr::launched("flow_tail_planes_bwd");
}

namespace {
int launch_pf_bwd(const float* grad_y, const float* wpk, float* G, int chunk0, int chunks, int B, int H, int W, int accumulate,
                  const PfFinalize& fin, hipStream_t st) {
  const long threads = (long)B * H * W * 4;
  const int bx = ufr::ceil_div(threads, 256);
  int slices = 1;
  while ((long)bx * slices < 1024 && slices < chunks) slices *= 2;
  if (slices > chunks) slices = chunks;
  const int per = ufr::ceil_div(chunks, slices);
  slices = ufr::ceil_div(chunks, per);
  (void)ufr::ensure_dynamic_lds(reinterpret_cast<const void*>(flow_head_planes_bwd), 48 * 576 * 4);
  flow_head_planes_bwd<<<dim3(bx, slices), 256, (size_t)per * 576 * 4, st>>>(grad_y, wpk, G, chunk0, chunks, B, H, W, accumulate, per, fin);
  return ufr::launched("flow_head_planes_bwd");
}
}

extern "C" int ufr_flow_head_planes_backward(const float* grad_y, const float* wpk, int w_chunks, float* G, int g_chunks, int chunk0,
                                             int chunks, int B, int H, int W, int accumulate, ufr_stream_t stream) {
  UFR_REQUIRE(grad_y && wpk && G, "flow head (planes) backward: null pointer");
  UFR_REQUIRE(B > 0 && H > 0 && W > 0 && chunks > 0 && chunks <= 48 && chunk0 >= 0 && (long)B * H * W < (1L << 29),
              "flow head (planes) backward: bad shape");
  UFR_REQUIRE_GRANGE("flow head (planes) backward", chunk0, chunks, w_chunks, g_chunks);
  return launch_pf_bwd(grad_y, wpk, G, chunk0, chunks, B, H, W, accumulate, PfFinalize{nullptr, nullptr, 0, 0, 0, 1.f}, ufr::as_stream(stream));
}

extern "C" int ufr_flow_head_planes_backward_finalize(const float* grad_y, const float* wpk, int w_chunks, float* G, int g_chunks,
                                                      int chunk0, int chunks, int B, int H, int W, int accumulate,
                                                      const void* mask_planes, void* out_planes, long out_plane_stride, int fin_chunk0,
                                                      int fin_chunks, float slope, ufr_stream_t stream) {
  UFR_REQUIRE(grad_y && wpk && G && out_planes, "flow head (planes) backward + finalize: null pointer");
  UFR_REQUIRE(B > 0 && H > 0 && W > 0 && chunks > 0 && chunks <= 48 && chunk0 >= 0 && (long)B * H * W < (1L << 29),
              "flow head (planes) backward + finalize: bad shape");
  UFR_REQUIRE_GRANGE("flow head (planes) backward + finalize", chunk0, chunks, w_chunks, g_chunks);
  UFR_REQUIRE(planes_hold(out_plane_stride, (long)B * H * W, chunk0 + fin_chunk0, fin_chunks),
              "flow head (planes) backward + finalize: the finalised segment leaves the gradient planes");
  UFR_REQUIRE(fin_chunk0 >= 0 && fin_chunks > 0 && fin_chunk0 + fin_chunks <= chunks && out_plane_stride > 0,
              "flow head (planes) backward + finalize: the finalised segment leaves the tensor");
  return launch_pf_bwd(grad_y, wpk, G, chunk0, chunks, B, H, W, accumulate,
                       PfFinalize{static_cast<const __bf16*>(mask_planes), static_cast<__bf16*>(out_planes), out_plane_stride, fin_chunk0,
                                  fin_chunks, slope},
// ... 68 lines not shown
```

understanding_flow_robustness_amd/flownetc_engine.py:

```python
from __future__ import annotations

import os

import torch
from ._lib import engine_cache as _engine_cache

from . import _lib as L
from . import igemm as ig

_HEADS = ((6, 1024), (5, 1026), (4, 770), (3, 386), (2, 194))


def _pack_flow_head(weight: torch.Tensor) -> torch.Tensor:
    cin = weight.shape[1]
    chunks = ig.pad32(cin) // 32
    w = torch.zeros(2, chunks * 32, 9, dtype=torch.float32, device=weight.device)
    w[:, :cin] = weight.detach().float().reshape(2, cin, 9)
    return w.view(2, chunks, 32, 9).permute(1, 3, 0, 2).contiguous()


def _pack_flow_head_mfma(weight: torch.Tensor) -> torch.Tensor:
    cin = weight.shape[1]
    chunks = ig.pad32(cin) // 32
    w = torch.zeros(chunks * 32, 32, dtype=torch.float32, device=weight.device)
    w[:cin, :18] = weight.detach().float().reshape(2, cin, 9).permute(1, 2, 0).reshape(cin, 18)
    wn = w.view(chunks, 32, 32).permute(0, 2, 1).contiguous()
    planes = ig._split3(wn).view(3, chunks, 32, 32).permute(1, 0, 2, 3).contiguous()
    return planes


def _pack_flow_tail_mfma(weight2: torch.Tensor) -> torch.Tensor:
    cout = weight2.shape[1]
    chunks = ig.pad32(cout) // 32
    w = torch.zeros(chunks * 32, 32, dtype=torch.float32, device=weight2.device)
    w[:cout] = weight2.detach().float().reshape(2, cout, 16).permute(1, 2, 0).reshape(cout, 32)
    wn = w.view(chunks, 32, 32).permute(0, 2, 1).contiguous()
    return ig._split3(wn).view(3, chunks, 32, 32).permute(1, 0, 2, 3).contiguous()


class FlowNetCHeadEngine:
    def __init__(self, net, B: int, H: int, W: int, device):
        if H % 64 or W % 64:
            raise ValueError("FlowNetC head engine: frame sides must be multiples of 64")
        L.lib()
        self.net, self.B, self.H, self.W, self.dev = net, int(B), int(H), int(W), torch.device(device)
        g = {s: (H // s, W // s) for s in (4, 8, 16, 32, 64)}
        self.grid = g
        P = lambda s, chunks: ig.Planes(B, g[s][0], g[s][1], chunks, self.dev)
        G = lambda s, chunks: ig.GradSum(B, g[s][0], g[s][1], chunks, self.dev)
        self.siamese = hasattr(net, "conv_redir")
        self.c3a_p, self.c3b_p = (P(8, 8), P(8, 8)) if self.siamese else (None, None)
        self.in31, self.cat3, self.cat2 = P(8, 15 if self.siamese else 8), P(8, 13), P(4, 7)
        self.c4a, self.cat4 = P(16, 16), P(16, 25)
        self.c5a, self.cat5 = P(32, 16), P(32, 33)
        self.c6a, self.c6 = P(64, 32), P(64, 32)
        f32 = dict(dtype=torch.float32, device=self.dev)
        self.flow = {k: torch.zeros(B, 2, *g[2 ** k], **f32) for k in (6, 5, 4, 3, 2)}
        self.G_cat2, self.G_cat3, self.G_cat4, self.G_cat5 = G(4, 7), G(8, 13), G(16, 25), G(32, 33)
        self.G_c6, self.G_in31, self.G_c3a = G(64, 32), G(8, 15 if self.siamese else 8), G(8, 8)
        self.gz_cat2, self.gz_cat3, self.gz_cat4, self.gz_cat5 = P(4, 7), P(8, 13), P(16, 25), P(32, 33)
        self.gz_c6, self.gz_c6a, self.gz_c5a, self.gz_c4a = P(64, 32), P(64, 32), P(32, 16), P(16, 16)
        self.gz_in31 = P(8, 15) if self.siamese else None
        self.g_flow = {k: torch.zeros(B, 2, *g[2 ** k], **f32) for k in (6, 5, 4, 3)}
        self.g_corr = torch.zeros(B, 21, 21, *g[8], **f32)
        self.g_c2a = torch.zeros(B, 128, *g[4], **f32)
        self.g_c3a, self.g_c3a_redir, self.g_c3b = (torch.zeros(B, 256, *g[8], **f32) for _ in range(3))
        self.c3_nchw = torch.zeros(2 * B, 256, *g[8], **f32)
        self._prefix = None
        self.flow_out, self.flow_scale = self.flow[2], float(getattr(net, "div_flow", 20.0))
        self._wprefixes, self._wprefix = {}, None
        self._win_m3 = 0
        self._build_launches()

    def _conv(self, name):
        return getattr(self.net, name)[0]

    def _bias(self, conv):
        if conv.bias is None:
            return torch.zeros(conv.out_channels, dtype=torch.float32, device=self.dev)
        return conv.bias.detach().float().contiguous()

    def _stem_layers(self):
        from .plane_graph import stem_stages
        return [(name, block[0], lvl) for lvl, stage in enumerate(stem_stages(self.net), 1) for name, block in stage]

    def _build_launches(self):
        net, g, B = self.net, self.grid, self.B
        plans = []

        def plan(wi, x, in_chunk0, rows, out_hw, **kw):
            M = B * rows[0] * rows[1]
            pk = [len(t) * wi.KC for _, _, t in wi.phases]
            kw.setdefault("variant", self._variant_for(wi))
            bm, target = self._tile_rows_and_slots(wi, kw)
            S = ig.splitk_for(M, wi.Npad, max(pk), len(wi.phases), phase_ktiles=pk, bm=bm, target=target)
            kw["variant"], S = ig.tuned(wi, M, kw, kw["variant"], S, rows=rows)
            plans.append((wi, x, in_chunk0, rows, out_hw, S, kw))
            return len(plans) - 1

        self._pipe_variant = {"0": 2, "5": 5}.get(os.environ.get("UFR_IGEMM_PIPE", "6"), 6)

        fwd, bwd = {}, {}
        cw = lambda n, s, p: ig.conv_forward_weights(self._conv(n).weight, s, p)
        cb = lambda n, s, p: ig.conv_backward_weights(self._conv(n).weight, s, p)
        bias = lambda n: self._bias(self._conv(n))
        if self.siamese:
            fwd["conv_redir"] = plan(cw("conv_redir", 1, 0), self.c3a_p, 0, g[8], g[8], out_planes=self.in31, out_chunk0=0,
                                     bias=bias("conv_redir"))
        fwd["conv3_1"] = plan(cw("conv3_1", 1, 1), self.in31, 0, g[8], g[8], out_planes=self.cat3, out_chunk0=0, bias=bias("conv3_1"))
        fwd["conv4"] = plan(cw("conv4", 2, 1), self.cat3, 0, g[16], g[16], out_planes=self.c4a, bias=bias("conv4"))
        fwd["conv4_1"] = plan(cw("conv4_1", 1, 1), self.c4a, 0, g[16], g[16], out_planes=self.cat4, out_chunk0=0, bias=bias("conv4_1"))
        fwd["conv5"] = plan(cw("conv5", 2, 1), self.cat4, 0, g[32], g[32], out_planes=self.c5a, bias=bias("conv5"))
        fwd["conv5_1"] = plan(cw("conv5_1", 1, 1), self.c5a, 0, g[32], g[32], out_planes=self.cat5, out_chunk0=0, bias=bias("conv5_1"))
        fwd["conv6"] = plan(cw("conv6", 2, 1), self.cat5, 0, g[64], g[64], out_planes=self.c6a, bias=bias("conv6"))
        fwd["conv6_1"] = plan(cw("conv6_1", 1, 1), self.c6a, 0, g[64], g[64], out_planes=self.c6, bias=bias("conv6_1"))
        dec = {5: (self.c6, 64, self.cat5, 16), 4: (self.cat5, 32, self.cat4, 16), 3: (self.cat4, 16, self.cat3, 8),
               2: (self.cat3, 8, self.cat2, 4)}
        for k, (src, s_in, dst, chunk0) in dec.items():
            n = f"deconv{k}"
            fwd[n] = plan(ig.deconv_forward_weights(self._conv(n).weight, 1), src, 0, g[s_in], g[s_in // 2], out_planes=dst,
                          out_chunk0=chunk0, bias=bias(n))
        gz = {5: (self.gz_cat5, 16, 16), 4: (self.gz_cat4, 16, 8), 3: (self.gz_cat3, 8, 4), 2: (self.gz_cat2, 4, 2)}
        Gabove = {2: self.G_cat3, 3: self.G_cat4, 4: self.G_cat5}
        self.tail_w, self.tail_args = {}, {}
        for k in (2, 3, 4):
            src, chunk0, _ = gz[k]
            s_in = {2: 8, 3: 16, 4: 32}[k]
            w = self._conv(f"deconv{k}").weight
            main = w.shape[0] - 2
            bwd[f"deconv{k}"] = plan(ig.deconv_backward_weights(w[:main], 1), src, chunk0, g[s_in], g[s_in], out_f32=Gabove[k])
            self.tail_w[k] = _pack_flow_tail_mfma(w[main:])
            self.tail_args[k] = (src, chunk0, ig.pad32(w.shape[1]) // 32, Gabove[k], main // 32, g[s_in])
        bwd["deconv5"] = plan(ig.deconv_backward_weights(self._conv("deconv5").weight, 1), self.gz_cat5, 16, g[64], g[64],
                              add=self.G_c6, mask=self.c6, out_planes=self.gz_c6)
        bwd["conv6_1"] = plan(cb("conv6_1", 1, 1), self.gz_c6, 0, g[64], g[64], mask=self.c6a, out_planes=self.gz_c6a)
        bwd["conv6"] = plan(cb("conv6", 2, 1), self.gz_c6a, 0, g[64], g[32], add=self.G_cat5, mask=self.cat5, out_planes=self.gz_cat5)
        bwd["conv5_1"] = plan(cb("conv5_1", 1, 1), self.gz_cat5, 0, g[32], g[32], mask=self.c5a, out_planes=self.gz_c5a)
        bwd["conv5"] = plan(cb("conv5", 2, 1), self.gz_c5a, 0, g[32], g[16], add=self.G_cat4, mask=self.cat4, out_planes=self.gz_cat4)
        bwd["conv4_1"] = plan(cb("conv4_1", 1, 1), self.gz_cat4, 0, g[16], g[16], mask=self.c4a, out_planes=self.gz_c4a)
        bwd["conv4"] = plan(cb("conv4", 2, 1), self.gz_c4a, 0, g[16], g[8], add=self.G_cat3, mask=self.cat3, out_planes=self.gz_cat3)
        if self.siamese:
            bwd["conv3_1"] = plan(cb("conv3_1", 1, 1), self.gz_cat3, 0, g[8], g[8], mask=self.in31, out_planes=self.gz_in31,
                                  out_f32=self.G_in31, planes_chunks=1, f32_first_chunk=1)
            bwd["conv_redir"] = plan(cb("conv_redir", 1, 0), self.gz_in31, 0, g[8], g[8], out_f32=self.G_c3a)
        else:
            bwd["conv3_1"] = plan(cb("conv3_1", 1, 1), self.gz_cat3, 0, g[8], g[8], out_f32=self.G_in31)
        need = max([len(wi.phases) * S * B * rows[0] * rows[1] * wi.Npad for wi, _, _, rows, _, S, _ in plans if S > 1] + [1])
        self.ws = torch.empty(need, dtype=torch.float32, device=self.dev)
        launches = [ig.make_launch(wi, x, c0, rows, out_hw, splitk=S, ws=self.ws if S > 1 else None, **kw)
                    for wi, x, c0, rows, out_hw, S, kw in plans]
        self.fwd = {k: launches[i] for k, i in fwd.items()}
        self.plain = {}
        self.bwd = {k: self._with_tail(("full", k), launches[i], plans[i][:5], plans[i][6], plans[i][5]) for k, i in bwd.items()}
        self._plans = {("fwd", k): plans[i] for k, i in fwd.items()}
        self._plans.update({("bwd", k): plans[i] for k, i in bwd.items()})
        self._band, self.fwd_band, self.bwd_band = None, {}, {}
        self.bwd_band_wide, self.bwd_rest, self._band_plans, self._pf_band, self._split_w = {}, {}, {}, {}, {}
        self.pf_w = {k: _pack_flow_head(getattr(net, f"predict_flow{k}").weight) for k, _ in _HEADS}
        self.pf_wm = {k: _pack_flow_head_mfma(getattr(net, f"predict_flow{k}").weight) for k, _ in _HEADS}
        self.pf_b = {k: getattr(net, f"predict_flow{k}").bias.detach().float().contiguous() for k, _ in _HEADS}
        self.up = {k: getattr(net, f"upsampled_flow{k}_to_{k - 1}") for k in (6, 5, 4, 3)}
        self.up_w = {k: m.weight.detach().float().contiguous() for k, m in self.up.items()}
        self.up_b = {k: (m.bias.detach().float().contiguous() if m.bias is not None else None) for k, m in self.up.items()}
        self.pf_src = {6: (self.c6, 32), 5: (self.cat5, 33), 4: (self.cat4, 25), 3: (self.cat3, 13), 2: (self.cat2, 7)}
        self.pf_G = {6: self.G_c6, 5: self.G_cat5, 4: self.G_cat4, 3: self.G_cat3, 2: self.G_cat2}
        self.up_dst = {6: (self.cat5, 32), 5: (self.cat4, 24), 4: (self.cat3, 12), 3: (self.cat2, 6)}
        self.up_G = {6: (self.G_cat5, 32), 5: (self.G_cat4, 24), 4: (self.G_cat3, 12), 3: (self.G_cat2, 6)}

    def _with_tail(self, key, plain, args, kw, S, resident=None):
        self.plain.pop(key, None)
        if S != 1 and resident is None:
            return plain
        wi, x, c0, rows, out_hw = args
        launch = ig.make_launch(wi, x, c0, rows, out_hw, ws=self.ws, balance=True, resident=resident, **kw)
        if launch.tail_plan is None:
            return plain
        self.plain[key] = plain
        return launch

    def tail_launches(self):
        tables = {"full": self.bwd, "band": self.bwd_band, "rest": self.bwd_rest}
        return [(tag, name, tables[tag][name].tail_plan) for tag, name in sorted(self.plain)]

    def _variant_for(self, wi):
        return self._pipe_variant if wi.Npad % 128 == 0 else 2

    @staticmethod
    def _tile_rows_and_slots(wi, kw):
        v = kw.get("variant", 0)
        if wi.Npad % 128:
            return 128, 768
        if v == 4:
            return 64, 1024
        if v == 5:
            return 128, 512
        if v == 6:
            return 256, 256
        return 128, 768

    def _build_prefix(self):
        B, dev = self.B, self.dev
        H, W = self.H, self.W
        layers = self._stem_layers()
        wis = [None] + [ig.conv_forward_weights(conv.weight, conv.stride[0], conv.padding[0]) for _, conv, _ in layers[1:]]
        scratch = {}

        def level_buffer(lvl, slot, chunks):
            if (lvl, slot) not in scratch:
                scratch[(lvl, slot)] = ig.Planes(B, H >> lvl, W >> lvl, chunks, dev)
            return scratch[(lvl, slot)]
        halves = {}
        for h, taps in (("a", {2: self.cat2, 3: self.c3a_p}), ("b", {3: self.c3b_p})):
            outs = []
            for i, (_, conv, lvl) in enumerate(layers):
                later = sum(1 for _, _, l in layers[i + 1:] if l == lvl)
                outs.append(taps[lvl] if later == 0 and lvl in taps else level_buffer(lvl, later % 2, ig.pad32(conv.out_channels) // 32))
            chain = []
            for i in range(1, len(layers)):
                name, conv, lvl = layers[i]
                launch = ig.make_launch(wis[i], outs[i - 1], 0, (H >> lvl, W >> lvl), (H >> lvl, W >> lvl), out_planes=outs[i],
                                        out_chunk0=0, bias=self._bias(conv), variant=self._variant_for(wis[i]))
                chain.append((name, launch, wis[i]))
            conv1 = layers[0][1]
            P = dict(c1=outs[0], layers=chain, b1=self._bias(conv1), w1=conv1.weight.detach())
            P.update({name: launch for name, launch, _ in chain})
            P.update({name + "_wi": wi for name, _, wi in chain})
            P.update(self._conv1_launch(B, H, W, outs[0]))
            halves[h] = P
        self._prefix = halves

    def _conv1_launch(self, n: int, H: int, W: int, c1: ig.Planes) -> dict:
        conv1 = self._stem_layers()[0][1]
        bias = self._bias(conv1)
        if os.environ.get("UFR_CONV1_DIRECT", "1") != "0":
            return dict(direct=dict(wimg=ig.conv1_direct_weights(conv1.weight), bias=bias, c1=c1, n=n, hw=(H, W),
                                    gflop=2.0 * n * (H // 2) * (W // 2) * 147 * 64 / 1e9))
        packed = ig.Planes(n, H // 2 + 3, W // 2 + 2, 1, self.dev)
        wi = ig.conv1_packed_weights(conv1.weight)
        launch = ig.make_launch(wi, packed, 0, (H // 2, W // 2), (H // 2, W // 2), out_planes=c1, bias=bias, variant=2)
        return dict(packed=packed, conv1=launch, conv1_wi=wi)

    def _conv1(self, P: dict, a: torch.Tensor, b: torch.Tensor | None):
        a = a.contiguous()
        L.require_hip(a, "frames")
        nb = 0 if b is None else int(b.shape[0])
        mean = self.net._mean64.reshape(-1).contiguous()
        D = P.get("direct")
        if D is not None:
            c1 = D["c1"]
            L.check(L.lib().ufr_conv1_direct(L.ptr(a), L.ptr(b.contiguous()) if b is not None else None, int(a.shape[0]), nb,
# ... 209 lines not shown
        for k, (lead, ls) in self._SPLIT_DECONV.items():
            src, chunk0, _, Gd, _, rows = self.tail_args[k]
            w = self._conv(f"deconv{k}").weight
            main, n_band = w.shape[0] - 2, self._conv(lead).out_channels
            if n_band % 32 or not 0 < n_band < main:
                continue
            name = f"deconv{k}"
            if name not in self._split_w:
                self._split_w[name] = (ig.deconv_backward_weights(w[:n_band], 1), ig.deconv_backward_weights(w[n_band:main], 1))
            w_band, w_rest = self._split_w[name]
            self.bwd_band[name] = planned(name, w_band, src, chunk0, (rows[0], band.width // ls), rows,
                                          dict(out_f32=Gd, out_f32_chunk0=0, row_band=(origin, 8, ls)))
            self.bwd_rest[name + " rest"] = planned(name + " rest", w_rest, src, chunk0, rows, rows,
                                                    dict(out_f32=Gd, out_f32_chunk0=n_band // 32))
            self._pf_band[k + 1] = (n_band // 32, ls)
        cw = int(getattr(band, "corr_width", 0))
        if cw:
            if cw % 8 or cw > band.width:
                raise ValueError("correlation band: a multiple of 8 pixels inside the band")
            for name in ("conv3_1", "conv_redir"):
                wi, x, c0, rows, out_hw, _, kw = self._plans[("bwd", name)]
                self.bwd_band_wide[name] = self.plain.get(("band", name), self.bwd_band[name])
                kw = dict(kw, row_band=(band.win[:, 2], 8, 8), in_band=(origin, 8, 8, band.width // 8))
                self.bwd_band[name] = planned(name, wi, x, c0, (rows[0], cw // 8), out_hw, kw)

    def replan(self, kind: str, name: str, tag: str):
        if kind == "bwd" and name in self._band_plans and tag == ("full" if name in self.bwd_rest else "band"):
            wi, x, c0, rows, out_hw, kw = self._band_plans[name]
            return wi, x, c0, rows, out_hw, dict(kw)
        wi, x, c0, rows, out_hw, _, kw = self._plans[(kind, name)]
        kw = dict(kw)
        if tag == "band":
            band = self._band
            ls_rows, ls_in = (self._FWD_BAND[name][0], None) if kind == "fwd" else self._BWD_BAND[name]
            origin = band.win[:, 1]
            rows = (rows[0], band.width // ls_rows)
            kw["row_band"] = (origin, 8, ls_rows)
            if ls_in is not None:
                kw["in_band"] = (origin, 8, ls_in, band.width // ls_in)
        return wi, x, c0, rows, out_hw, kw

    def launch_table(self):
        rows = []
        for kind, table, tag in (("fwd", self.fwd, "full"), ("bwd", self.bwd, "full"), ("fwd", self.fwd_band, "band"),
                                 ("bwd", self.bwd_band, "band"), ("bwd", self.bwd_rest, "full")):
            for name, launch in table.items():
                wi = self._band_plans[name][0] if kind == "bwd" and table is not self.bwd and name in self._band_plans else \
                    self._plans[(kind, name)][0]
                d = launch.desc
                rows.append((name, kind, tag, launch, wi.flops(d.B * d.Hr * d.Wr) / 1e9))
        if self._prefix is not None:
            for h, suffix in (("a", ""), ("b", " 2nd frames")):
                F = self._prefix[h]
                packed = [("conv1", F["conv1"], F["conv1_wi"])] if "conv1" in F else []
                for key, launch, wi in packed + F["layers"]:
                    d = launch.desc
                    rows.append((key + suffix, "fwd", "prefix", launch, wi.flops(d.B * d.Hr * d.Wr) / 1e9))
        P = getattr(self, "_wprefix", None)
        if P is not None:
            packed = [("conv1", P["conv1"], P["conv1_wi"])] if "conv1" in P else []
            for kind, chain in (("fwd", packed + P["fwd"]), ("bwd", P["bwd"])):
                for key, launch, wi in chain:
                    d = launch.desc
                    rows.append((key[:-4] if kind == "bwd" else key, kind, "window", launch, wi.flops(d.B * d.Hr * d.Wr) / 1e9))
        return rows

    def conv1_direct_table(self):
        rows = []
        sets = []
        if self._prefix is not None:
            sets += [("conv1 direct" + sfx, "prefix", self._prefix[h]) for h, sfx in (("a", ""), ("b", " 2nd frames"))]
        if getattr(self, "_wprefix", None) is not None:
            sets.append(("conv1 direct", "window", self._wprefix))
        for label, tag, P in sets:
            D = P.get("direct")
            if D is None:
                continue
            n, (H, W) = D["n"], D["hw"]
            frames = torch.rand(n, 3, H, W, device=self.dev)
            nbytes = n * 3 * H * W * 4 + n * (H // 2) * (W // 2) * 64 * 6
            rows.append((label, tag, (lambda P=P, frames=frames: self._conv1(P, frames, None)), float(nbytes), D["gflop"]))
        return rows

    def _pf_forward(self, k):
        src, chunks = self.pf_src[k]
        L.check(L.lib().ufr_flow_head_planes_forward_mfma(L.ptr(src.t), src.plane_stride, 0, chunks, L.ptr(self.pf_wm[k]),
                                                          self.pf_wm[k].shape[0], L.ptr(self.pf_b[k]), L.ptr(self.flow[k]), self.B, src.H, src.W,
                                                          L.stream()), "predict_flow forward (mfma)")

    def _pf_backward(self, k, gy, accumulate, finalize=None, region=None):
        src, chunks = self.pf_src[k]
        if region is not None:
            head, kind, origin, stride, div, rh, rw, margin, wout = region
            act, out, c0, n = finalize if finalize is not None else (None, None, 0, 0)
            L.check(L.lib().ufr_flow_head_planes_backward_regions(
                L.ptr(gy), L.ptr(self.pf_w[k]), self.pf_w[k].shape[0], L.ptr(self.pf_G[k].t), self.pf_G[k].chunks, 0, chunks, self.B,
                src.H, src.W, int(accumulate), int(head), int(kind), L.ptr(origin), int(stride), int(div), int(rh), int(rw), int(margin),
                L.ptr(wout.t) if wout is not None else None, wout.B if wout is not None else 0,
                L.ptr(act.t) if act is not None else None, L.ptr(out.t) if out is not None else None,
                out.plane_stride if out is not None else 0, int(c0), int(n), float(ig.LEAKY), L.stream()),
                "predict_flow backward (regions)")
            return
        if finalize is not None:
            act, out, c0, n = finalize
            L.check(L.lib().ufr_flow_head_planes_backward_finalize(L.ptr(gy), L.ptr(self.pf_w[k]), self.pf_w[k].shape[0], L.ptr(self.pf_G[k].t),
                                                                   self.pf_G[k].chunks, 0, chunks, self.B,
                                                                   src.H, src.W, int(accumulate), L.ptr(act.t), L.ptr(out.t), out.plane_stride,
                                                                   int(c0), int(n), float(ig.LEAKY), L.stream()),
                    "predict_flow backward + finalize")
            return
        L.check(L.lib().ufr_flow_head_planes_backward(L.ptr(gy), L.ptr(self.pf_w[k]), self.pf_w[k].shape[0], L.ptr(self.pf_G[k].t),
                                                      self.pf_G[k].chunks, 0, chunks, self.B,
                                                      src.H, src.W, int(accumulate), L.stream()), "predict_flow backward")

    def _up_forward(self, k):
        dst, chunk = self.up_dst[k]
        f = self.flow[k]
        L.check(L.lib().ufr_flow_up_planes_forward(L.ptr(f), L.ptr(self.up_w[k]), L.ptr(self.up_b[k]) if self.up_b[k] is not None else None,
                                                   L.ptr(dst.t), dst.plane_stride, chunk, self.B, f.shape[2], f.shape[3],
                                                   L.stream()), "upsampled_flow forward")

    def _deconv_tail(self, k):
        src, chunk0, chunks, Gd, out_chunk, (h, w) = self.tail_args[k]
        L.check(L.lib().ufr_deconv_flow_tail_backward_mfma(L.ptr(src.t), src.plane_stride, chunk0, chunks, L.ptr(self.tail_w[k]),
                                                           self.tail_w[k].shape[0], L.ptr(Gd.t), Gd.chunks, out_chunk, self.B, h, w, L.stream()),
                "deconv data gradient, flow channels")

    def _up_backward(self, k):
        G, chunk = self.up_G[k]
        f = self.g_flow[k]
        L.check(L.lib().ufr_flow_up_planes_backward(L.ptr(G.t), chunk, L.ptr(self.up_w[k]), L.ptr(f), self.B, f.shape[2],
                                                    f.shape[3], 0, L.stream()), "upsampled_flow backward")

    def _finalize(self, Gs, mask, out, chunk0, chunks):
        L.check(L.lib().ufr_grad_finalize(L.ptr(Gs.t), chunk0, L.ptr(mask.t), chunk0, L.ptr(out.t), out.plane_stride, chunk0,
                                          Gs.M, chunks, ig.LEAKY, L.stream()), "gradient finalize")

    def _forward_trunk(self, c2: torch.Tensor, c3: torch.Tensor) -> torch.Tensor:
        L.require_hip(c2, "c2")
        L.require_hip(c3, "c3")
        self.cat2.load_nchw(c2, 0)
        self.in31.load_nchw(c3, 0)
        for name in ("conv3_1", "conv4", "conv4_1", "conv5", "conv5_1", "conv6", "conv6_1"):
            self.fwd[name]()
        self._pf_forward(6)
        for k in (5, 4, 3, 2):
            self._up_forward(k + 1)
            self.fwd[f"deconv{k}"]()
            self._pf_forward(k)
        return self.flow[2]

    def forward_cached(self, band=None, corr_changed: bool = True) -> torch.Tensor:
        return self.forward(None, self._c3a, self._c3b, band, corr_changed=corr_changed)

    def forward(self, c2a: torch.Tensor | None, c3a: torch.Tensor, c3b: torch.Tensor, band=None,
                corr_changed: bool = True) -> torch.Tensor:
        if not self.siamese:
            return self._forward_trunk(c2a, c3a)
        for t, name in ((c3a, "c3a"), (c3b, "c3b")):
            L.require_hip(t, name)
        self._c3a, self._c3b = c3a, c3b
        inc = False
        if band is not None:
            self.attach_band(band)
            inc = bool(band.width and band.incremental and band.inc_layers)
        if c2a is not None:
            L.require_hip(c2a, "c2a")
            self.cat2.load_nchw(c2a, 0)
            self.c3a_p.load_nchw(c3a, 0)
            self.c3b_p.load_nchw(c3b, 0)
        if inc and band.cone_win is not None and band.cone_hw[1] // 8 <= 23:
            if corr_changed:
                L.check(L.lib().ufr_corr_forward_planes_changed(L.ptr(self.c3a_p.t), L.ptr(self.c3b_p.t), self.c3a_p.plane_stride,
                                                                L.ptr(self.in31.t), self.in31.plane_stride, 1, self.B, 256, *self.grid[8],
                                                                21, 2, 1.0 / 256.0, ig.LEAKY, L.ptr(band.cone_win), 8,
                                                                band.cone_hw[0] // 8, band.cone_hw[1] // 8, self._win_m3, L.stream()),
                        "correlation forward (planes, changed)")
            else:
                L.check(L.lib().ufr_corr_forward_planes_window(L.ptr(self.c3a_p.t), L.ptr(self.c3b_p.t), self.c3a_p.plane_stride,
                                                               L.ptr(self.in31.t), self.in31.plane_stride, 1, self.B, 256, *self.grid[8],
                                                               21, 2, 1.0 / 256.0, ig.LEAKY, L.ptr(band.cone_win), 8,
                                                               band.cone_hw[1] // 8, L.stream()), "correlation forward (planes, window)")
        else:
            L.check(L.lib().ufr_corr_forward_planes(L.ptr(self.c3a_p.t), L.ptr(self.c3b_p.t), self.c3a_p.plane_stride,
                                                    L.ptr(self.in31.t), self.in31.plane_stride, 1, self.B, 256, *self.grid[8], 21, 2,
                                                    1.0 / 256.0, ig.LEAKY, L.stream()), "correlation forward (planes)")
        for name in ("conv_redir", "conv3_1", "conv4", "conv4_1"):
            (self.fwd_band if inc else self.fwd)[name]()
        for name in ("conv5", "conv5_1", "conv6", "conv6_1"):
            self.fwd[name]()
        self._pf_forward(6)
        for k in (5, 4, 3, 2):
            self._up_forward(k + 1)
            self.fwd[f"deconv{k}"]()
            self._pf_forward(k)
        return self.flow[2]

    def backward(self, g_flow2: torch.Tensor, band=None, fused_window: bool = True, skip_unread: bool = True, tail_split: bool = True):
        L.require_hip(g_flow2, "g_flow2")
        B = self.B
        run = lambda table, tag, name: (table[name] if tail_split else self.plain.get((tag, name), table[name]))()
        banded = band is not None and bool(band.width)
        if band is not None:
            self.attach_band(band)
        gz = {2: (self.G_cat2, self.cat2, self.gz_cat2, 4, 2), 3: (self.G_cat3, self.cat3, self.gz_cat3, 8, 4),
              4: (self.G_cat4, self.cat4, self.gz_cat4, 16, 8), 5: (self.G_cat5, self.cat5, self.gz_cat5, 16, 16)}
        fuse = os.environ.get("UFR_FUSE_FINALIZE", "1") != "0"
        fin = lambda k: (gz[k][1], gz[k][2], gz[k][3], gz[k][4]) if fuse else None
        eng_window = bool(fused_window and band is not None and getattr(band, "eng_window", False)
                          and getattr(self, "_wprefix", None) is not None)
        skip = bool(skip_unread and banded and fused_window and self.siamese)
        if skip and eng_window:
            P = self._wprefix
            wh, ww = P["hw"]
            self._pf_backward(2, g_flow2, accumulate=False, finalize=fin(2),
                              region=(4, L.UFR_PF_REGION_WINDOW, band.cone_win, 8, 4, wh // 4, ww // 4, band.g2_margin, P["G_gw2"]))
        else:
            self._pf_backward(2, g_flow2, accumulate=False, finalize=fin(2))
            if eng_window:
                self.window_gather_conv2_gradient(band.cone_win, band.g2_margin)
            else:
                self.G_cat2.to_nchw(128, 0, out=self.g_c2a)
        for k in (2, 3, 4):
            Gs, act, out, chunk0, chunks = gz[k]
            if not fuse:
                self._finalize(Gs, act, out, chunk0, chunks)
            self._up_backward(k + 1)
            region = None
            if skip and k + 1 in self._pf_band:
                run(self.bwd_band, "band", f"deconv{k}")
                run(self.bwd_rest, "rest", f"deconv{k} rest")
                head, ls = self._pf_band[k + 1]
                region = (head, L.UFR_PF_REGION_BAND, band.win[:, 1], 8, ls, self.grid[ls][0], band.width // ls, 0, None)
            else:
                run(self.bwd, "full", f"deconv{k}")
            self._deconv_tail(k)
            self._pf_backward(k + 1, self.g_flow[k + 1], accumulate=True, finalize=fin(k + 1), region=region)
        Gs, act, out, chunk0, chunks = gz[5]
        if not fuse:
            self._finalize(Gs, act, out, chunk0, chunks)
        self._up_backward(6)
        self._pf_backward(6, self.g_flow[6], accumulate=False)
        for name in ("deconv5", "conv6_1", "conv6", "conv5_1"):
            run(self.bwd, "full", name)
        if not self.siamese:
            for name in ("conv5", "conv4_1", "conv4", "conv3_1"):
                run(self.bwd, "full", name)
            self.G_in31.to_nchw(256, 0, out=self.g_c3a)
            return self.g_c2a, self.g_c3a, None
        for name in ("conv5", "conv4_1", "conv4", "conv3_1", "conv_redir"):
            if banded and not skip and name in self.bwd_band_wide:
                self.bwd_band_wide[name]()
            elif banded:
                run(self.bwd_band, "band", name)
            else:
                run(self.bwd, "full", name)
        gw = getattr(band, "g3_window", None) if (band is not None and fused_window) else None
        h8, w8 = self.grid[8]
        if gw is not None and band.cone_win is not None and band.cone_hw[1] // 8 <= 16 and w8 % 4 == 0:
            L.check(L.lib().ufr_corr_backward_window_fused(L.ptr(self._c3a), L.ptr(self._c3b), L.ptr(self.G_in31.t), 1, 1.0 / 256.0,
                                                           L.ptr(self.G_c3a.t), L.ptr(gw), B, 256, h8, w8, 21, 2,
                                                           L.ptr(band.cone_win), 8, band.cone_hw[0] // 8, band.cone_hw[1] // 8,
                                                           int(band.g3_margin), L.stream()), "correlation backward (window, fused)")
            return (None if eng_window else self.g_c2a), None, None
        self.G_c3a.to_nchw(256, 0, out=self.g_c3a_redir)
        self.G_in31.to_nchw(441, 1, scale=1.0 / 256.0, out=self.g_corr.view(B, 441, *self.grid[8]))
        self._corr_backward(self.g_corr, band)
        return (None if eng_window else self.g_c2a), self.g_c3a, self.g_c3b

    def _corr_backward(self, g_corr, band):
        from . import spatial_correlation_sampler_backend as correlation
        import ctypes as C
        h8, w8 = self.grid[8]
        if band is not None and band.cone_win is not None:
            L.check(L.lib().ufr_corr_backward_window(L.ptr(self._c3a), L.ptr(self._c3b), L.ptr(g_corr), L.ptr(self.g_c3a),
                                                     L.ptr(self.g_c3b), self.B, 256, h8, w8, 21, 2, L.ptr(band.cone_win), 8,
                                                     band.cone_hw[0] // 8, band.cone_hw[1] // 8, L.stream()),
                    "correlation backward (window)")
        else:
            p = correlation._params(1, 1, 21, 21, 0, 0, 1, 1, 2, 2, 1, 1)
            L.check(L.lib().ufr_corr_backward(L.ptr(self._c3a), L.ptr(self._c3b), L.ptr(g_corr), L.ptr(self.g_c3a),
                                              L.ptr(self.g_c3b), L.UFR_F32, self.B, 256, h8, w8, C.byref(p), L.stream()),
                    "correlation backward")
        self.g_c3a.add_(self.g_c3a_redir)

    REPLACEABLE = ("conv3a", "conv3b", "corr", "conv_redir", "conv3_1")
    _HEAD_SEGMENTS = {
        "conv_redir": ("in31", 0, 32), "corr": ("in31", 1, 441), "conv3_1": ("cat3", 0, 256), "deconv3": ("cat3", 8, 128),
        "upsampled_flow4_to_3": ("cat3", 12, 2), "conv4": ("c4a", 0, 512), "conv4_1": ("cat4", 0, 512), "deconv4": ("cat4", 16, 256),
        "upsampled_flow5_to_4": ("cat4", 24, 2), "conv5": ("c5a", 0, 512), "conv5_1": ("cat5", 0, 512), "deconv5": ("cat5", 16, 512),
        "upsampled_flow6_to_5": ("cat5", 32, 2), "conv6": ("c6a", 0, 1024), "conv6_1": ("c6", 0, 1024), "deconv2": ("cat2", 4, 64),
        "upsampled_flow3_to_2": ("cat2", 6, 2)}
    _FLOW_KEYS = {"flow6": 6, "flow5": 5, "flow4": 4, "flow3": 3, "predict": 2}

    def segment_map(self, stem=None) -> dict:
        if not self.siamese:
            raise RuntimeError("feature-map segments: the FlowNetC head (the FlowNetS trunk has no correlation)")
        seg = {}
        if stem is not None:
            for lvl, cn in ((1, 64), (2, 128), (3, 256)):
                p = stem.bufs[f"c{lvl}"].planes
                seg[f"conv{lvl}a"], seg[f"conv{lvl}b"] = (p, 0, cn, 0, None), (p, 0, cn, self.B, None)
        for key, (buf, c0, cn) in self._HEAD_SEGMENTS.items():
            seg[key] = (getattr(self, buf), c0, cn, 0, "unleaky" if key == "corr" else None)
        for key, k in self._FLOW_KEYS.items():
            seg[key] = (self.flow[k], 0, 2, 0, None)
        return seg

    def capture(self, keys=None, stem=None) -> dict:
        seg = self.segment_map(stem)
        out = {}
        for key in (list(seg) if keys is None else keys):
            if key not in seg:
                raise KeyError(f"capture: {key!r} is not a feature map of this forward ({', '.join(seg)})")
            src, c0, cn, img0, post = seg[key]
            if isinstance(src, ig.Planes):
                t = src.to_nchw(cn, c0)[img0:img0 + self.B]
                out[key] = _unleaky(t, ig.LEAKY) if post == "unleaky" else (t if t.shape[0] == src.B else t.clone())
            else:
                out[key] = src[:, c0:c0 + cn].clone()
        return out

    def forward_replaced(self, c2a, c3a, c3b, overwrite=None, keep=(), computed=None) -> torch.Tensor:
        if not self.siamese:
            raise RuntimeError("feature-map replacement: the FlowNetC head")
        ow = {k: v for k, v in (overwrite or {}).items() if k in self.REPLACEABLE}
        keep = {k for k in keep if k in self.REPLACEABLE and k not in ow}
        pair = lambda d: "conv3a" in d and "conv3b" in d
        for t, name in ((c2a, "c2a"), (c3a, "c3a"), (c3b, "c3b")):
            L.require_hip(t, name)
        self.generation = getattr(self, "generation", 0) + 1
        self._c3a, self._c3b = c3a, c3b
        self.cat2.load_nchw(c2a, 0)
        if pair(ow):
            self.c3a_p.load_nchw(ow["conv3a"].contiguous(), 0)
            self.c3b_p.load_nchw(ow["conv3b"].contiguous(), 0)
        elif not pair(keep):
            self.c3a_p.load_nchw(c3a, 0)
            self.c3b_p.load_nchw(c3b, 0)

        def stage(key, launch, load):
            if key not in ow and key not in keep:
                launch()
                return
            if computed is not None:
                held = self.capture([key]) if key in keep else None
                launch()
                computed[key] = self.capture([key])[key]
                if held is not None:
                    load(held[key])
            if key in ow:
                load(ow[key].contiguous())

        corr = lambda: L.check(L.lib().ufr_corr_forward_planes(
            L.ptr(self.c3a_p.t), L.ptr(self.c3b_p.t), self.c3a_p.plane_stride, L.ptr(self.in31.t), self.in31.plane_stride, 1, self.B,
            256, *self.grid[8], 21, 2, 1.0 / 256.0, ig.LEAKY, L.stream()), "correlation forward (planes)")
        stage("corr", corr, lambda v: self.in31.load_nchw(v, 1, slope=ig.LEAKY))
        stage("conv_redir", self.fwd["conv_redir"], lambda v: self.in31.load_nchw(v, 0))
        stage("conv3_1", self.fwd["conv3_1"], lambda v: self.cat3.load_nchw(v, 0))
        for name in ("conv4", "conv4_1", "conv5", "conv5_1", "conv6", "conv6_1"):
            self.fwd[name]()
        self._pf_forward(6)
        for k in (5, 4, 3, 2):
            self._up_forward(k + 1)
            self.fwd[f"deconv{k}"]()
            self._pf_forward(k)
        return self.flow[2]


def _unleaky(x: torch.Tensor, slope: float) -> torch.Tensor:
    s = torch.tensor(slope, dtype=torch.float32, device=x.device)
    y0 = x / s
    best, found = y0.clone(), x >= 0
    bits = y0.view(torch.int32)
    for d in (-2, -1, 0, 1, 2):
        cand = (bits + d).view(torch.float32)
        ok = ~found & (cand * s == x)
        best = torch.where(ok, cand, best)
        found = found | ok
    return torch.where(x < 0, best, x)


class _EngineHead(torch.autograd.Function):

    @staticmethod
    def forward(ctx, c2a, c3a, c3b, engine, band):
        ctx.engine, ctx.band = engine, band
        engine.generation = ctx.generation = getattr(engine, "generation", 0) + 1
        ctx.static, ctx.static_grads = L.static_ok(), L.static_grads_ok()
        flow2 = engine.forward(c2a.contiguous(), c3a.contiguous(), c3b.contiguous() if c3b is not None else None, band)
        return flow2.detach() if ctx.static else flow2.clone()

    @staticmethod
    def backward(ctx, g_flow2):
        if ctx.engine.generation != ctx.generation:
            raise RuntimeError("FlowNetC head engine: another forward of this network (same batch and frame size) ran before this "
                               "backward; its activations are gone.  Call backward() before the next forward, or set "
                               "UFR_ENGINE=0 for interleaved forwards")
        g2a, g3a, g3b = ctx.engine.backward(g_flow2.contiguous(), ctx.band, fused_window=False)
        if ctx.static_grads:
            return g2a, g3a, g3b, None, None
        return (g2a.clone() if g2a is not None else None, g3a.clone() if g3a is not None else None,
                g3b.clone() if g3b is not None else None, None, None)


def _weights_stamp(net):
    return tuple((p.data_ptr(), p._version) for p in net.parameters())


def get_engine(net, B: int, H: int, W: int, device) -> FlowNetCHeadEngine:
    key = (int(B), int(H), int(W), str(torch.device(device)))
    cache = _engine_cache(net, "_ufr_head_engines")
    stamp = _weights_stamp(net)
    eng = cache.get(key)
    if eng is None or eng.weights_stamp != stamp:
        eng = cache[key] = FlowNetCHeadEngine(net, B, H, W, device)
        eng.weights_stamp = stamp
    return eng


def engine_head(net, c2a, c3a, c3b, band=None):
    B, _, h4, w4 = c2a.shape
    return _EngineHead.apply(c2a, c3a, c3b, get_engine(net, B, h4 * 4, w4 * 4, c2a.device), band)
```

understanding_flow_robustness_amd/patch_attack.py:

```python
from __future__ import annotations

import ctypes as C
import os
from argparse import Namespace

import numpy as np
import torch
from ._lib import engine_cache as _engine_cache

from . import _lib as L
from .flownets.utils_model import predict_flow

LOSS_THRESHOLD = 0.1
CLAMP_BOUND = 2.0


def _pixel_range(flownet: str):
    return (0.0, 1.0) if any(k in flownet for k in ("FlowNetC", "FlowNetS", "FlowNet2", "RAFT", "PWC")) else (-1.0, 1.0)


class ShardedExchange:

    def __init__(self, group=None):
        import torch.distributed as dist
# ... 239 lines not shown
                self.eng.prefix_full(self.adv_tgt.detach(), self.adv_ref.detach())
            return
        feats = prefix_features if prefix_features is not None else \
            self.net.encode(torch.cat((self.adv_tgt.detach(), self.adv_ref.detach()), 0))
        for (ls, m, n, full, _), f in zip(self.taps, feats):
            if f.shape[0] < n or f.shape[1:] != full.shape[1:]:
                raise ValueError("prefix_features do not match this step's frames")
            full.detach().copy_(f[:n])

    def _forward_cone(self):
        lib, B, H, W = L.lib(), self.B, self.H, self.W
        wh, ww = self.win_hw
        L.check(lib.ufr_window_gather_pair(L.ptr(self.adv_tgt), L.ptr(self.adv_ref), L.ptr(self.xw), L.ptr(self.win),
                                           L.ptr(self.loss_local), B, 3, H, W, wh, ww, L.stream()), "window gather (pair)")
        if self.eng is not None:
            self._feats_w = None
            if self.eng_kind == "pwc":
                self.eng.window_prefix_forward(self.xw, self.win, self.taps[0][1])
                self.eng.forward_cached()
            else:
                (_, m2, _, _, _), (_, m3, _, _, _) = self.taps
                self.eng.window_prefix_forward(self.xw, self.win, m2, m3, c2_nchw=False)
                self.eng.forward_cached(self.band, corr_changed=self.corr_changed)
            if self._fused_loss:
                return None
            return torch.nn.functional.interpolate(self.eng.flow_out * self.eng.flow_scale, scale_factor=4, mode="bilinear",
                                                   align_corners=False)
        self._feats_w = [f[:n] for f, (_, _, n, _, _) in zip(self.net.encode(self.xw), self.taps)]
        for f, (ls, m, n, full, _) in zip(self._feats_w, self.taps):
            self._win_copy(lib.ufr_window_scatter, f, full, n, f.shape[1], H // ls, W // ls, ls, m)
        full = [t[3] for t in self.taps]
        extra = {"band": self.band} if self.band is not None else {}
        return self.net.head(*full[:-1], full[-1][:B], full[-1][B:], **extra)

    def _backward_cone(self, flow):
        lib, B, H, W = L.lib(), self.B, self.H, self.W
        self._packed_grad = False
        if self.eng is not None:
            if flow is None:
                g_flow2 = self.g_flow2
            else:
                (g_flow2,) = torch.autograd.grad(flow, (self.eng.flow_out,), self.g_flow)
            if self.eng_kind == "pwc":
                ls, m, n, _, gw = self.taps[0]
                g_f2 = self.eng.backward(g_flow2.contiguous())
                self._win_copy(lib.ufr_window_gather, g_f2, gw, n, g_f2.shape[1], H // ls, W // ls, ls, m)
                gxw = self.eng.window_prefix_backward(gw)
            else:
                (ls2, m2, _, _, gw2), (ls3, m3, _, _, gw3) = self.taps
                if self.band is not None:
                    self.band.g3_window, self.band.g3_margin = gw3, m3
                    self.band.eng_window, self.band.g2_margin = True, m2
                g2a, g3a, g3b = self.eng.backward(g_flow2.contiguous(), self.band, skip_unread=self.skip_unread,
                                                  tail_split=self.tail_split)
                if g2a is not None:
                    self._win_copy(lib.ufr_window_gather, g2a, gw2, B, 128, H // ls2, W // ls2, ls2, m2)
                if g3a is not None:
                    self._win_copy(lib.ufr_window_gather, g3a, gw3, B, 256, H // ls3, W // ls3, ls3, m3)
                    self._win_copy(lib.ufr_window_gather, g3b, gw3[B:], B, 256, H // ls3, W // ls3, ls3, m3)
                self._packed_grad = self.placed
                gxw = self.eng.window_prefix_backward(self.taps[1][4], None if g2a is None else self.taps[0][4],
                                                      unpack=not self.placed)
        else:
            g_full = torch.autograd.grad(flow, [t[3] for t in self.taps], self.g_flow)
            for g, (ls, m, n, _, gwin) in zip(g_full, self.taps):
                self._win_copy(lib.ufr_window_gather, g.contiguous(), gwin, n, g.shape[1], H // ls, W // ls, ls, m)
            gxw, = torch.autograd.grad(self._feats_w, (self.xw,), [t[4] for t in self.taps])
        self._feats_w = None
        gxw = gxw.contiguous()
        if self.placed:
            return gxw, None
        self._win_copy(lib.ufr_window_scatter, gxw, self.g_tgt_full, B, 3, H, W, 1, 0)
        self._win_copy(lib.ufr_window_scatter, gxw[B:], self.g_ref_full, B, 3, H, W, 1, 0)
        return self.g_tgt_full, self.g_ref_full

    def _part_a(self):
        if self.cone is not None:
            flow = self._forward_cone()
        else:
            self.loss_local.zero_()
            flow = predict_flow(self.net, None, self.adv_tgt, self.adv_ref, self.args)
        weight = (1.0 - self.alpha) * ((1.0 / self.world) if self.shared else float(self.B))
        if flow is None:
            L.check(L.lib().ufr_flow2_upsampled_loss(L.ptr(self.eng.flow_out), float(self.eng.flow_scale), L.ptr(self.target),
                                                     L.ptr(self.g_flow2), L.ptr(self.loss_local), self.B, self.H // 4, self.W // 4,
                                                     self.kind, weight, L.ptr(self.loss_ws), L.stream()), "upsampled flow loss")
        else:
            if not flow.is_contiguous():
                flow = flow.contiguous()
            L.check(L.lib().ufr_flow_loss(L.ptr(flow), L.ptr(self.target), L.ptr(self.g_flow), L.ptr(self.loss_local),
                                          self.B, self.H * self.W, self.kind, weight, L.ptr(self.loss_ws), L.stream()),
                    "flow loss")
        if not self.shared:
            self.loss_local.div_(float(self.B))
        if self.alpha != 0.0:
            if self.placed:
                reg = (self.mask_p * self.patch - self.mask_p * self.patch_init).abs().sum() / float(self.CHW)
            else:
                reg = torch.nn.functional.l1_loss(self.mask * self.patch, self.mask * self.patch_init)
            self.loss_local.add_(self.alpha * reg / self.world)
        if self.cone is not None:
            g_tgt, g_ref = self._backward_cone(flow)
        else:
            g_tgt, g_ref = torch.autograd.grad(flow, (self.adv_tgt, self.adv_ref), self.g_flow)
            g_tgt, g_ref = g_tgt.contiguous(), g_ref.contiguous()
        if not self.placed:
            self._update(g_tgt, g_ref)
            self._gate()
            return
        if g_ref is None:
            wh, ww = self.win_hw
            crop = L.lib().ufr_patch_grad_crop_packed if self._packed_grad else L.lib().ufr_patch_grad_crop_window
            L.check(crop(L.ptr(g_tgt), L.ptr(self.win), L.ptr(self.mask_p), L.ptr(self.origins),
                                                       L.ptr(self.loss_local), L.ptr(self.rows_local), self.B, self.H, self.W, wh, ww,
                                                       self.ph, self.pw, self.groups, L.stream()), "patch grad crop (window)")
        else:
            self._crop(g_tgt, g_ref)
        if self.world == 1:
            self._apply()
            self._gate()

    def _part_b(self):
        self._apply()
        self._gate()

    def _gate(self):
        L.check(L.lib().ufr_attack_gate(L.ptr(self.loss_cur), L.ptr(self.state), LOSS_THRESHOLD, L.stream()),
                "attack gate")

    def _incremental_now(self):
        band = getattr(self, "band", None)
        return bool(self.cone is not None and band is not None and band.inc_layers and not self._first)

    def _set_later(self, later: bool):
        band = getattr(self, "band", None) if self.cone is not None else None
        if band is not None:
            band.incremental = bool(later and band.inc_layers)
        self._rect_paste = bool(later and self.placed and os.environ.get("UFR_RECT_PASTE", "1") != "0")

    def _iteration(self):
        later = not self._first
        if self.graph is not None:
            (self.graph_next if later else self.graph).replay()
        else:
            self._set_later(later)
            self._part_a()
        self._first = False
        if self.world > 1:
            self.exchange.gather(self.rows_local, self.rows_all)
            if self.graph_b is not None:
                (self.graph_b_next if later else self.graph_b).replay()
            else:
                self._part_b()
        if self.graph is None:
            self._set_later(False)

    def _capture(self):
        side = torch.cuda.Stream(device=self.dev)
        side.wait_stream(torch.cuda.current_stream(self.dev))
        with torch.cuda.stream(side):
            for _ in range(max(self._warmup, 2)):
                self._iteration()
        torch.cuda.current_stream(self.dev).wait_stream(side)
        torch.cuda.synchronize(self.dev)
        if not self.use_graph:
            return
        graphs = {}
        for later in (False, True):
            self._set_later(later)
# ... 260 lines not shown
```

Baseline: 1533.

## Split-K flow head GEMM with fused finish/upsample, and faster upsampled flow loss

Adds a split-over-channels MFMA kernel for the predict_flow heads when the plan reports too few tiles to fill the GPU. Per-slice partials are then reduced by a finish kernel that also adds the bias, does the 3x3 tap sum and fuses the 2x flow upsampling into the planes write. The forward path now defers the finish so it can merge with the following upsample step. Separately, the upsampled flow loss switches to a new tiled shared-memory kernel that computes the loss and the gradient with a gather back to flow2. These changes trade extra partial-buffer traffic and more complex code for better occupancy and fewer launches.

After: 1556 (median of 6 runs). 1.5% higher.

```diff
diff --git a/include/ufr_hip.h b/include/ufr_hip.h
--- a/include/ufr_hip.h
+++ b/include/ufr_hip.h
@@ -161,6 +161,8 @@
                   int HW, int kind, float weight, float* partials, ufr_stream_t stream);
 int ufr_flow2_upsampled_loss(const float* flow2, float flow_scale, const float* target, float* grad_flow2, float* loss, int B,
                              int h, int w, int kind, float weight, float* partials, ufr_stream_t stream);
+int ufr_flow2_upsampled_loss_fast(const float* flow2, float flow_scale, const float* target, float* grad_flow2, float* loss, int B,
+                                  int h, int w, int kind, float weight, float* partials, ufr_stream_t stream);
 
 int ufr_gru_gates_forward(const float* zr_pre, const float* h, float* z_out, float* rh_out, int B, int Ch,
                           int HW, long rh_bstride, ufr_stream_t stream);
@@ -422,6 +424,12 @@
                                  const float* bias, float* out, int B, int H, int W, ufr_stream_t stream);
 int ufr_flow_head_planes_forward_mfma(const void* planes, long plane_stride, int chunk0, int chunks, const void* wmf, int w_chunks,
                                       const float* bias, float* out, int B, int H, int W, ufr_stream_t stream);
+int ufr_flow_head_split_plan(int B, int H, int W, int chunks, int* slices, int* starved, long* partial_floats);
+int ufr_flow_head_planes_forward_split(const void* planes, long plane_stride, int chunk0, int chunks, const void* wmf, int w_chunks,
+                                       float* partials, long partial_floats, int slices, int B, int H, int W, ufr_stream_t stream);
+int ufr_flow_head_split_finish(const float* partials, long partial_floats, int slices, const float* bias, float* flow,
+                               const float* up_w, const float* up_bias, void* up_planes, long up_plane_stride, int up_chunk, int B,
+                               int H, int W, ufr_stream_t stream);
 int ufr_deconv_flow_tail_backward_mfma(const void* grad_planes, long plane_stride, int chunk0, int chunks, const void* wmf,
                                        int w_chunks, float* G, int g_chunks, int out_chunk, int B, int H, int W, ufr_stream_t stream);
 int ufr_flow_head_planes_backward(const float* grad_y, const float* wpk, int w_chunks, float* G, int g_chunks, int chunk0, int chunks,
diff --git a/understanding_flow_robustness_amd/_lib.py b/understanding_flow_robustness_amd/_lib.py
--- a/understanding_flow_robustness_amd/_lib.py
+++ b/understanding_flow_robustness_amd/_lib.py
@@ -155,6 +155,7 @@
                              _i, _vp],
     "ufr_flow_loss": [_vp, _vp, _vp, _vp, _i, _i, _i, _f, _vp, _vp],
     "ufr_flow2_upsampled_loss": [_vp, _f, _vp, _vp, _vp, _i, _i, _i, _i, _f, _vp, _vp],
+    "ufr_flow2_upsampled_loss_fast": [_vp, _f, _vp, _vp, _vp, _i, _i, _i, _i, _f, _vp, _vp],
     "ufr_patch_grad_crop": [_vp, _vp, _vp, _vp, _vp, _vp, _vp, _i, _i, _i, _i, _i, _i, _vp],
     "ufr_patch_apply": [_vp, _i, _vp, _vp, _i, _i, _f, _f, _vp, _vp],
     "ufr_patch_grad_crop_window": [_vp, _vp, _vp, _vp, _vp, _vp, _i, _i, _i, _i, _i, _i, _i, _i, _vp],
@@ -246,6 +247,9 @@
     "ufr_upfeat_planes_forward_mfma": [_vp, _l, _i, _i, _vp, _i, _vp, _vp, _i, _i, _i, _vp],
     "ufr_upfeat_planes_backward": [_vp, _vp, _i, _vp, _i, _i, _i, _i, _i, _i, _i, _vp],
     "ufr_flow_up_planes_forward": [_vp, _vp, _vp, _vp, _l, _i, _i, _i, _i, _vp],
+    "ufr_flow_head_split_plan": [_i, _i, _i, _i, C.POINTER(C.c_int), C.POINTER(C.c_int), C.POINTER(C.c_long)],
+    "ufr_flow_head_planes_forward_split": [_vp, _l, _i, _i, _vp, _i, _vp, _l, _i, _i, _i, _i, _vp],
+    "ufr_flow_head_split_finish": [_vp, _l, _i, _vp, _vp, _vp, _vp, _vp, _l, _i, _i, _i, _i, _vp],
     "ufr_flow_up_planes_backward": [_vp, _i, _vp, _vp, _i, _i, _i, _i, _vp],
     "ufr_corr_forward_planes_changed": [_vp, _vp, _l, _vp, _l, _i, _i, _i, _i, _i, _i, _i, _f, _f, _vp, _i, _i, _i, _i, _vp],
     "ufr_corr_forward_planes_window": [_vp, _vp, _l, _vp, _l, _i, _i, _i, _i, _i, _i, _i, _f, _f, _vp, _i, _i, _vp],
diff --git a/understanding_flow_robustness_amd/csrc/attack.hip b/understanding_flow_robustness_amd/csrc/attack.hip
--- a/understanding_flow_robustness_amd/csrc/attack.hip
+++ b/understanding_flow_robustness_amd/csrc/attack.hip
@@ -529,6 +529,159 @@
   return ufr::launched("flow2_upsampled_loss_kernel");
 }
 
+constexpr int F2_G = 4 * F2_T + 4, F2_C = F2_T + 2;
+__global__ __launch_bounds__(256) void flow2_upsampled_loss_fast_kernel(const float* __restrict__ flow2, float flow_scale,
+                                                                        const float* __restrict__ target,
+                                                                        float* __restrict__ gflow2, float* __restrict__ partials,
+                                                                        int B, int h, int w, int kind, float weight) {
+  __shared__ float f2[2][F2_C][F2_C];
+  __shared__ float g[2][F2_G][F2_G];
+  __shared__ float tl[2][F2_G];
+  __shared__ unsigned char ti[2][2][F2_G];
+  __shared__ float red[4];
+  const int tid = threadIdx.x, b = blockIdx.z;
+  const int cy0 = blockIdx.y * F2_T, cx0 = blockIdx.x * F2_T;
+  const int H = 4 * h, W = 4 * w;
+  const long HW = (long)H * W, hw = (long)h * w;
+  const float invn = weight / (float)((long)B * HW);
+  for (int i = tid; i < 2 * F2_C * F2_C; i += 256) {
+    const int c = i / (F2_C * F2_C), r = i - c * F2_C * F2_C, yy = r / F2_C, xx = r - yy * F2_C;
+    const int cy = min(max(cy0 - 1 + yy, 0), h - 1), cx = min(max(cx0 - 1 + xx, 0), w - 1);
+    f2[c][yy][xx] = flow2[((long)b * 2 + c) * hw + (long)cy * w + cx] * flow_scale;
+  }
+  if (tid < 2 * F2_G) {
+    const int axis = tid / F2_G, r = tid - axis * F2_G;
+    const int c0 = axis ? cx0 : cy0, n = axis ? w : h, p = 4 * c0 - 2 + r;
+    int i0 = 255 + c0 - 1, i1 = 255 + c0 - 1;
+    float l1 = 0.f;
+    if (p >= 0 && p < 4 * n) up4_source(p, n, i0, i1, l1);
+    ti[axis][0][r] = (unsigned char)(i0 - (c0 - 1));
+    ti[axis][1][r] = (unsigned char)(i1 - (c0 - 1));
+    tl[axis][r] = l1;
+  }
+  __syncthreads();
+  const int py0 = 4 * cy0 - 2, px0 = 4 * cx0 - 2;
+  float part = 0.f;
+  int ry = tid / F2_R, rx = tid - ry * F2_R;
+  constexpr int F2_K = (F2_R * F2_R + 255) / 256;
+  for (int k0 = 0; k0 < F2_K; k0 += 3) {
+    int gy[3], gx[3];
+    bool store[3], live[3], owned[3];
+    float tu[3], tv[3];
+#pragma unroll
+    for (int j = 0; j < 3; ++j) {
+      gy[j] = ry - 2;
+      gx[j] = rx - 2;
+      store[j] = ry < F2_R && gy[j] >= 0 && gy[j] < F2_G && gx[j] >= 0 && gx[j] < F2_G;
+      live[j] = store[j] && ti[0][0][store[j] ? gy[j] : 0] != 255 && ti[1][0][store[j] ? gx[j] : 0] != 255;
+      owned[j] = ry >= 4 && ry < F2_R - 4 && rx >= 4 && rx < F2_R - 4;
+      tu[j] = tv[j] = 0.f;
+      if (live[j]) {
+        const long o0 = ((long)b * 2) * HW + (long)(py0 + gy[j]) * W + (px0 + gx[j]);
+        tu[j] = target[o0];
+        tv[j] = target[o0 + HW];
+      }
+      rx += 256 - 3 * F2_R;
+      ry += 3;
+      if (rx >= F2_R) { rx -= F2_R; ++ry; }
+    }
+#pragma unroll
+    for (int j = 0; j < 3; ++j) {
+      float gu = 0.f, gv = 0.f;
+      if (live[j]) {
+        const int a0 = ti[0][0][gy[j]], a1 = ti[0][1][gy[j]], c0 = ti[1][0][gx[j]], c1 = ti[1][1][gx[j]];
+        const float ly = tl[0][gy[j]], lx = tl[1][gx[j]];
+        const float hy0 = 1.f - ly, wx0 = 1.f - lx;
+        const float fu = hy0 * (wx0 * f2[0][a0][c0] + lx * f2[0][a0][c1]) + ly * (wx0 * f2[0][a1][c0] + lx * f2[0][a1][c1]);
+        const float fv = hy0 * (wx0 * f2[1][a0][c0] + lx * f2[1][a0][c1]) + ly * (wx0 * f2[1][a1][c0] + lx * f2[1][a1][c1]);
+        const float tuj = tu[j], tvj = tv[j];
+        float term;
+        if (kind == 0) {
+          const float dot = fu * tuj + fv * tvj;
+          const float nf2 = fu * fu + fv * fv, nt2 = tuj * tuj + tvj * tvj;
+          const float den = fmaxf(sqrtf(nf2 * nt2), 1e-8f);
+          const float c = dot / den;
+          term = 1.0f - c;
+          if (sqrtf(nf2 * nt2) > 1e-8f) {
+            gu = -(tuj / den - c * fu / nf2);
+            gv = -(tvj / den - c * fv / nf2);
+          } else {
+            gu = -(tuj / den);
+            gv = -(tvj / den);
+          }
+        } else {
+          const float du = fu - tuj, dv = fv - tvj;
+          const float sd = sqrtf(du * du + dv * dv + 1e-8f);
+          term = sd;
+          gu = du / sd;
+          gv = dv / sd;
+        }
+        gu *= invn;
+        gv *= invn;
+        if (owned[j]) part += term;
+      }
+      if (store[j]) {
+        g[0][gy[j]][gx[j]] = gu;
+        g[1][gy[j]][gx[j]] = gv;
+      }
+    }
+  }
+  __syncthreads();
+  {
+    const int cyl = tid >> 4, cxl = tid & 15, cy = cy0 + cyl, cx = cx0 + cxl;
+    if (cy < h && cx < w) {
+      float wxs[8];
+      bool vx[8];
+#pragma unroll
+      for (int t = 0; t < 8; ++t) {
+        const int c = 4 * cxl + t, x0 = ti[1][0][c], x1 = ti[1][1][c];
+        const float lx = tl[1][c];
+        vx[t] = x0 != 255;
+        wxs[t] = (x0 == cxl + 1 ? 1.f - lx : 0.f) + (x1 == cxl + 1 ? lx : 0.f);
+      }
+      float su = 0.f, sv = 0.f;
+#pragma unroll
+      for (int s = 0; s < 8; ++s) {
+        const int r = 4 * cyl + s, y0 = ti[0][0][r], y1 = ti[0][1][r];
+        if (y0 == 255) continue;
+        const float ly = tl[0][r];
+        const float wy = (y0 == cyl + 1 ? 1.f - ly : 0.f) + (y1 == cyl + 1 ? ly : 0.f);
+        if (wy == 0.f) continue;
+        float ru = 0.f, rv = 0.f;
+#pragma unroll
+        for (int t = 0; t < 8; ++t)
+          if (vx[t]) {
+            ru += wxs[t] * g[0][r][4 * cxl + t];
+            rv += wxs[t] * g[1][r][4 * cxl + t];
+          }
+        su += wy * ru;
+        sv += wy * rv;
+      }
+      gflow2[((long)b * 2) * hw + (long)cy * w + cx] = su * flow_scale;
+      gflow2[((long)b * 2 + 1) * hw + (long)cy * w + cx] = sv * flow_scale;
+    }
+  }
+  for (int off = 32; off > 0; off >>= 1) part += __shfl_down(part, off, 64);
+  if ((tid & 63) == 0) red[tid >> 6] = part;
+  __syncthreads();
+  if (tid == 0) partials[(blockIdx.z * gridDim.y + blockIdx.y) * gridDim.x + blockIdx.x] = (red[0] + red[1] + red[2] + red[3]) * invn;
+}
+
+extern "C" int ufr_flow2_upsampled_loss_fast(const float* flow2, float flow_scale, const float* target, float* grad_flow2, float* loss,
+                                             int B, int h, int w, int kind, float weight, float* partials, ufr_stream_t stream) {
+  UFR_REQUIRE(flow2 && target && grad_flow2 && loss && partials, "upsampled flow loss (fast): null pointer argument");
+  UFR_REQUIRE(B > 0 && h > 0 && w > 0 && (kind == 0 || kind == 1), "upsampled flow loss (fast): bad argument");
+  const dim3 grid(ufr::ceil_div(w, F2_T), ufr::ceil_div(h, F2_T), B);
+  const long n = (long)grid.x * grid.y * grid.z;
+  if (n > UFR_LOSS_PARTIALS || B > 65535)
+    return ufr::fail(UFR_EUNSUPPORTED, "upsampled flow loss (fast): %ld tiles exceed the %d partial sums of the fixed-order reduction", n,
+                     UFR_LOSS_PARTIALS);
+  hipLaunchKernelGGL(flow2_upsampled_loss_fast_kernel, grid, dim3(256), 0, ufr::as_stream(stream), flow2, flow_scale, target,
+                     grad_flow2, partials, B, h, w, kind, weight);
+  hipLaunchKernelGGL(loss_finalize_kernel, dim3(1), dim3(64), 0, ufr::as_stream(stream), partials, (int)n, loss);
+  return ufr::launched("flow2_upsampled_loss_fast_kernel");
+}
+
 namespace ufr {
 void loss_finalize_launch(const float* partials, int n, float* loss, hipStream_t st) {
   hipLaunchKernelGGL(loss_finalize_kernel, dim3(1), dim3(64), 0, st, partials, n, loss);
diff --git a/understanding_flow_robustness_amd/csrc/engine_small.hip b/understanding_flow_robustness_amd/csrc/engine_small.hip
--- a/understanding_flow_robustness_amd/csrc/engine_small.hip
+++ b/understanding_flow_robustness_amd/csrc/engine_small.hip
@@ -291,6 +291,132 @@
         o[1] = r1;
       }
     }
+  }
+}
+
+constexpr int PFS_TS = 18;
+__global__ __launch_bounds__(256) void flow_head_split_gemm(const __bf16* __restrict__ x, long plane_stride, int chunk0, int chunks,
+                                                            const __bf16* __restrict__ wmf, float* __restrict__ Tp, long M, int per) {
+  const int lane = threadIdx.x & 63, wave = threadIdx.x >> 6, slice = blockIdx.y;
+  const long m0 = ((long)blockIdx.x * 4 + wave) * 16;
+  if (m0 >= M) return;
+  const long p = m0 + (lane & 15);
+  const bool ok = p < M;
+  const __bf16* a = ok ? x + ((long)chunk0 * M + p) * 32 + (lane >> 4) * 8 : reinterpret_cast<const __bf16*>(pf_zero_page);
+  const long astep = ok ? M * 32 : 0;
+  const long pstep = ok ? plane_stride : 0;
+  const __bf16* wl = wmf + (lane & 15) * 32 + (lane >> 4) * 8;
+  const int c_lo = slice * per, c_hi = min(chunks, c_lo + per);
+  f32x4 acc[2] = {f32x4{0.f, 0.f, 0.f, 0.f}, f32x4{0.f, 0.f, 0.f, 0.f}};
+  bf16x8 fa[2][3], fb[2][2][3];
+  auto fetch = [&](int st, int ch) {
+#pragma unroll
+    for (int pl = 0; pl < 3; ++pl) {
+      fa[st][pl] = *reinterpret_cast<const bf16x8*>(a + (long)ch * astep + pl * pstep);
+#pragma unroll
+      for (int nt = 0; nt < 2; ++nt) fb[st][nt][pl] = *reinterpret_cast<const bf16x8*>(wl + (((long)ch * 3 + pl) * 2 + nt) * 512);
+    }
+  };
+  auto mma = [&](int st) {
+#pragma unroll
+    for (int nt = 0; nt < 2; ++nt)
+#pragma unroll
+      for (int q = 0; q < 6; ++q)
+        acc[nt] = __builtin_amdgcn_mfma_f32_16x16x32_bf16(fa[st][PFM_A[q]], fb[st][nt][PFM_B[q]], acc[nt], 0, 0, 0);
+  };
+  if (c_lo < c_hi) fetch(0, c_lo);
+  for (int ch = c_lo; ch < c_hi; ch += 2) {
+    if (ch + 1 < c_hi) fetch(1, ch + 1);
+    mma(0);
+    if (ch + 1 < c_hi) {
+      if (ch + 2 < c_hi) fetch(0, ch + 2);
+      mma(1);
+    }
+  }
+  float* T = Tp + ((long)slice * M + m0 + (lane >> 4) * 4) * PFS_TS;
+#pragma unroll
+  for (int r = 0; r < 4; ++r)
+    if (m0 + (lane >> 4) * 4 + r < M) {
+      T[r * PFS_TS + (lane & 15)] = acc[0][r];
+      if ((lane & 15) < 2) T[r * PFS_TS + 16 + (lane & 15)] = acc[1][r];
+    }
+}
+
+constexpr int PFF_T = 8;
+__global__ __launch_bounds__(256) void flow_head_split_finish(const float* __restrict__ Tp, int S, const float* __restrict__ bias,
+                                                              float* __restrict__ flow, const float* __restrict__ w,
+                                                              const float* __restrict__ up_bias, __bf16* __restrict__ planes,
+                                                              long plane_stride, int chunk, int B, int H, int W) {
+  __shared__ float f[2][PFF_T + 2][PFF_T + 2];
+  const int tid = threadIdx.x, b = blockIdx.z, cy0 = blockIdx.y * PFF_T, cx0 = blockIdx.x * PFF_T;
+  const long M = (long)B * H * W, HW = (long)H * W;
+  if (tid < (PFF_T + 2) * (PFF_T + 2)) {
+    const int hy = tid / (PFF_T + 2), hx = tid - hy * (PFF_T + 2), yy = cy0 - 1 + hy, xx = cx0 - 1 + hx;
+    float r0 = 0.f, r1 = 0.f;
+    if (yy >= 0 && yy < H && xx >= 0 && xx < W) {
+      int off[9];
+      unsigned inside = 0;
+#pragma unroll
+      for (int k = 0; k < 9; ++k) {
+        const int y2 = yy + k / 3 - 1, x2 = xx + k % 3 - 1;
+        const bool ok = y2 >= 0 && y2 < H && x2 >= 0 && x2 < W;
+        off[k] = ((ok ? y2 : yy) * W + (ok ? x2 : xx)) * PFS_TS + 2 * k;
+        inside |= ok ? 1u << k : 0u;
+      }
+      for (int sl = 0; sl < S; ++sl) {
+        const float* Ts = Tp + ((long)sl * M + (long)b * HW) * PFS_TS;
+        float2 e[9];
+#pragma unroll
+        for (int k = 0; k < 9; ++k) e[k] = *reinterpret_cast<const float2*>(Ts + off[k]);
+#pragma unroll
+        for (int k = 0; k < 9; ++k) {
+          r0 += (inside >> k & 1u) ? e[k].x : 0.f;
+          r1 += (inside >> k & 1u) ? e[k].y : 0.f;
+        }
+      }
+      r0 += bias[0];
+      r1 += bias[1];
+      if (hy >= 1 && hy <= PFF_T && hx >= 1 && hx <= PFF_T) {
+        flow[((long)b * 2 + 0) * HW + (long)yy * W + xx] = r0;
+        flow[((long)b * 2 + 1) * HW + (long)yy * W + xx] = r1;
+      }
+    }
+    f[0][hy][hx] = r0;
+    f[1][hy][hx] = r1;
+  }
+  if (!planes) return;
+  __syncthreads();
+  const int Ho = 2 * H, Wo = 2 * W;
+  const int Y = 2 * cy0 + (tid >> 4), X = 2 * cx0 + (tid & 15);
+  if (Y >= Ho || X >= Wo) return;
+  float a0 = up_bias ? up_bias[0] : 0.f, a1 = up_bias ? up_bias[1] : 0.f;
+#pragma unroll
+  for (int t = 0; t < 2; ++t) {
+    const int ky = ((Y + 1) & 1) + 2 * t, yy = (Y + 1 - ky) / 2;
+    if (Y + 1 - ky < 0 || yy >= H) continue;
+#pragma unroll
+    for (int u = 0; u < 2; ++u) {
+      const int kx = ((X + 1) & 1) + 2 * u, xx = (X + 1 - kx) / 2;
+      if (X + 1 - kx < 0 || xx >= W) continue;
+#pragma unroll
+      for (int ic = 0; ic < 2; ++ic) {
+        const float v = f[ic][yy - cy0 + 1][xx - cx0 + 1];
+        a0 = fmaf(v, w[((ic * 2 + 0) * 4 + ky) * 4 + kx], a0);
+        a1 = fmaf(v, w[((ic * 2 + 1) * 4 + ky) * 4 + kx], a1);
+      }
+    }
+  }
+  __bf16 s0[3], s1[3];
+  split3(a0, s0[0], s0[1], s0[2]);
+  split3(a1, s1[0], s1[1], s1[2]);
+  const long total = (long)B * Ho * Wo;
+  __bf16* dst = planes + ((long)chunk * total + ((long)b * Ho + Y) * Wo + X) * 32;
+#pragma unroll
+  for (int p = 0; p < 3; ++p) {
+    bf16x8 v = {s0[p], s1[p], (__bf16)0.f, (__bf16)0.f, (__bf16)0.f, (__bf16)0.f, (__bf16)0.f, (__bf16)0.f};
+    const bf16x8 zero = {(__bf16)0.f, (__bf16)0.f, (__bf16)0.f, (__bf16)0.f, (__bf16)0.f, (__bf16)0.f, (__bf16)0.f, (__bf16)0.f};
+    bf16x8* o = reinterpret_cast<bf16x8*>(dst + p * plane_stride);
+    o[0] = v; o[1] = zero; o[2] = zero; o[3] = zero;
   }
 }
 
@@ -632,6 +758,20 @@
 }
 
 namespace {
+struct PfMode0Plan { int TH, blocks, S; bool eight, starved; };
+PfMode0Plan pf_mode0_plan(int B, int H, int W, int chunks) {
+  auto blocks_of = [&](int th) { return (long)B * ufr::ceil_div(H, th) * ufr::ceil_div(W, 32); };
+  PfMode0Plan p;
+  p.TH = blocks_of(8) >= 512 ? 8 : (blocks_of(4) >= 256 ? 4 : 2);
+  p.blocks = (int)blocks_of(p.TH);
+  const int S = (p.blocks >= 512 || chunks < 4) ? 1 : 2;
+  const int mt = ((p.TH + 2) * 34 + 15) / 16;
+  p.eight = mt <= 12 && S == 2 && chunks >= 16 && p.blocks <= 256;
+  p.S = p.eight ? 8 : S;
+  p.starved = blocks_of(4) < 256;
+  return p;
+}
+
 template <int MODE>
 int launch_pf_mfma(const void* planes, long plane_stride, int chunk0, int chunks, const void* wmf, const float* bias, float* out,
                    int out_chunk, int B, int H, int W, hipStream_t st, const char* what) {
@@ -672,6 +812,52 @@
   UFR_REQUIRE_RANGE("flow head (planes, mfma) forward", plane_stride, (long)B * H * W, chunk0, chunks, w_chunks);
   return launch_pf_mfma<0>(planes, plane_stride, chunk0, chunks, wmf, bias, out, 0, B, H, W, ufr::as_stream(stream),
                            "flow_head_planes_fwd_mfma");
+}
+
+extern "C" int ufr_flow_head_split_plan(int B, int H, int W, int chunks, int* slices, int* starved, long* partial_floats) {
+  UFR_REQUIRE(slices && starved && partial_floats, "flow head split plan: null pointer");
+  UFR_REQUIRE(B > 0 && H > 0 && W > 0 && chunks > 0 && chunks <= 48 && (long)B * H * W < (1L << 29), "flow head split plan: bad shape");
+  const PfMode0Plan p = pf_mode0_plan(B, H, W, chunks);
+  *slices = p.S;
+  *starved = p.starved ? 1 : 0;
+  *partial_floats = (long)p.S * B * H * W * PFS_TS;
+  return UFR_OK;
+}
+
+extern "C" int ufr_flow_head_planes_forward_split(const void* planes, long plane_stride, int chunk0, int chunks, const void* wmf,
+                                                  int w_chunks, float* partials, long partial_floats, int slices, int B, int H, int W,
+                                                  ufr_stream_t stream) {
+  UFR_REQUIRE(planes && wmf && partials, "flow head (planes, split) forward: null pointer");
+  UFR_REQUIRE(B > 0 && H > 0 && W > 0 && chunks > 0 && chunks <= 48 && chunk0 >= 0 && (long)B * H * W < (1L << 29),
+              "flow head (planes, split) forward: bad shape");
+  UFR_REQUIRE_RANGE("flow head (planes, split) forward", plane_stride, (long)B * H * W, chunk0, chunks, w_chunks);
+  const PfMode0Plan p = pf_mode0_plan(B, H, W, chunks);
+  UFR_REQUIRE(slices == p.S, "flow head (planes, split) forward: %d chunk slices asked, the unsplit form of this grid adds %d (the sums "
+              "would differ in the last bits)", slices, p.S);
+  const long M = (long)B * H * W;
+  UFR_REQUIRE(partial_floats >= (long)slices * M * PFS_TS, "flow head (planes, split) forward: the partials buffer holds %ld floats, "
+              "%d slices of %ld pixels need %ld", partial_floats, slices, M, (long)slices * M * PFS_TS);
+  const int per = ufr::ceil_div(chunks, slices);
+  flow_head_split_gemm<<<dim3(ufr::ceil_div(M, 64), slices), 256, 0, ufr::as_stream(stream)>>>(
+      static_cast<const __bf16*>(planes), plane_stride, chunk0, chunks, static_cast<const __bf16*>(wmf), partials, M, per);
+  return ufr::launched("flow_head_split_gemm");
+}
+
+extern "C" int ufr_flow_head_split_finish(const float* partials, long partial_floats, int slices, const float* bias, float* flow,
+                                          const float* up_w, const float* up_bias, void* up_planes, long up_plane_stride, int up_chunk,
+                                          int B, int H, int W, ufr_stream_t stream) {
+  UFR_REQUIRE(partials && bias && flow, "flow head split finish: null pointer");
+  UFR_REQUIRE(B > 0 && B <= 65535 && H > 0 && W > 0 && slices > 0 && (long)B * H * W < (1L << 27), "flow head split finish: bad shape");
+  UFR_REQUIRE(partial_floats >= (long)slices * B * H * W * PFS_TS, "flow head split finish: the partials buffer holds %ld floats, %d "
+              "slices need %ld", partial_floats, slices, (long)slices * B * H * W * PFS_TS);
+  if (up_planes) {
+    UFR_REQUIRE(up_w && up_chunk >= 0, "flow head split finish: the upsampling needs its weights and a chunk");
+    UFR_REQUIRE(planes_hold(up_plane_stride, (long)B * H * W * 4, up_chunk, 1), "flow head split finish: chunk %d leaves the planes "
+                "operand", up_chunk);
+  }
+  flow_head_split_finish<<<dim3(ufr::ceil_div(W, PFF_T), ufr::ceil_div(H, PFF_T), B), 256, 0, ufr::as_stream(stream)>>>(
+      partials, slices, bias, flow, up_w, up_bias, static_cast<__bf16*>(up_planes), up_plane_stride, up_chunk, B, H, W);
+  return ufr::launched("flow_head_split_finish");
 }
 
 extern "C" int ufr_deconv_flow_tail_backward_mfma(const void* grad_planes, long plane_stride, int chunk0, int chunks, const void* wmf,
diff --git a/understanding_flow_robustness_amd/flownetc_engine.py b/understanding_flow_robustness_amd/flownetc_engine.py
--- a/understanding_flow_robustness_amd/flownetc_engine.py
+++ b/understanding_flow_robustness_amd/flownetc_engine.py
@@ -9,6 +9,14 @@
 from . import igemm as ig
 
 _HEADS = ((6, 1024), (5, 1026), (4, 770), (3, 386), (2, 194))
+
+
+def pf_split_plan(B: int, H: int, W: int, chunks: int):
+    import ctypes
+    slices, starved, floats = ctypes.c_int(0), ctypes.c_int(0), ctypes.c_long(0)
+    L.check(L.lib().ufr_flow_head_split_plan(int(B), int(H), int(W), int(chunks), ctypes.byref(slices), ctypes.byref(starved),
+                                             ctypes.byref(floats)), "predict_flow split plan")
+    return slices.value, bool(starved.value), floats.value
 
 
 def _pack_flow_head(weight: torch.Tensor) -> torch.Tensor:
@@ -166,6 +174,16 @@
         self.pf_G = {6: self.G_c6, 5: self.G_cat5, 4: self.G_cat4, 3: self.G_cat3, 2: self.G_cat2}
         self.up_dst = {6: (self.cat5, 32), 5: (self.cat4, 24), 4: (self.cat3, 12), 3: (self.cat2, 6)}
         self.up_G = {6: (self.G_cat5, 32), 5: (self.G_cat4, 24), 4: (self.G_cat3, 12), 3: (self.G_cat2, 6)}
+        self.pf_split, floats = {}, 0
+        for k in (6, 5, 4, 3):
+            src, chunks = self.pf_src[k]
+            slices, starved, n = pf_split_plan(self.B, src.H, src.W, chunks)
+            if starved:
+                self.pf_split[k] = (slices, n)
+                floats = max(floats, n)
+        self.pf_partials = torch.empty(max(floats, 1), dtype=torch.float32, device=self.dev)
+        self._pf_pending = None
+        self.pf_ran = {}
 
     def _with_tail(self, key, plain, args, kw, S, resident=None):
         self.plain.pop(key, None)
@@ -541,8 +559,19 @@
             rows.append((label, tag, (lambda P=P, frames=frames: self._conv1(P, frames, None)), float(nbytes), D["gflop"]))
         return rows
 
-    def _pf_forward(self, k):
+    def _pf_forward(self, k, defer=False):
         src, chunks = self.pf_src[k]
+        if k in self.pf_split:
+            slices, n = self.pf_split[k]
+            L.check(L.lib().ufr_flow_head_planes_forward_split(L.ptr(src.t), src.plane_stride, 0, chunks, L.ptr(self.pf_wm[k]),
+                                                               self.pf_wm[k].shape[0], L.ptr(self.pf_partials), n, slices, self.B, src.H,
+                                                               src.W, L.stream()), "predict_flow forward (split)")
+            self.pf_ran[k] = "split"
+            self._pf_pending = k
+            if not defer:
+                self._pf_finish(k, upsample=False)
+            return
+        self.pf_ran[k] = "mfma"
         L.check(L.lib().ufr_flow_head_planes_forward_mfma(L.ptr(src.t), src.plane_stride, 0, chunks, L.ptr(self.pf_wm[k]),
                                                           self.pf_wm[k].shape[0], L.ptr(self.pf_b[k]), L.ptr(self.flow[k]), self.B, src.H, src.W,
                                                           L.stream()), "predict_flow forward (mfma)")
@@ -572,7 +601,20 @@
                                                       self.pf_G[k].chunks, 0, chunks, self.B,
                                                       src.H, src.W, int(accumulate), L.stream()), "predict_flow backward")
 
+    def _pf_finish(self, k, upsample):
+        slices, n = self.pf_split[k]
+        f = self.flow[k]
+        dst, chunk = self.up_dst[k] if upsample else (None, 0)
+        L.check(L.lib().ufr_flow_head_split_finish(L.ptr(self.pf_partials), n, slices, L.ptr(self.pf_b[k]), L.ptr(f), L.ptr(self.up_w[k]),
+                                                   L.ptr(self.up_b[k]) if self.up_b[k] is not None else None,
+                                                   L.ptr(dst.t) if upsample else None, dst.plane_stride if upsample else 0, chunk, self.B,
+                                                   f.shape[2], f.shape[3], L.stream()), "predict_flow finish (split)")
+        self._pf_pending = None
+
     def _up_forward(self, k):
+        if self._pf_pending == k:
+            self._pf_finish(k, upsample=True)
+            return
         dst, chunk = self.up_dst[k]
         f = self.flow[k]
         L.check(L.lib().ufr_flow_up_planes_forward(L.ptr(f), L.ptr(self.up_w[k]), L.ptr(self.up_b[k]) if self.up_b[k] is not None else None,
@@ -602,11 +644,11 @@
         self.in31.load_nchw(c3, 0)
         for name in ("conv3_1", "conv4", "conv4_1", "conv5", "conv5_1", "conv6", "conv6_1"):
             self.fwd[name]()
-        self._pf_forward(6)
+        self._pf_forward(6, defer=True)
         for k in (5, 4, 3, 2):
             self._up_forward(k + 1)
             self.fwd[f"deconv{k}"]()
-            self._pf_forward(k)
+            self._pf_forward(k, defer=True)
         return self.flow[2]
 
     def forward_cached(self, band=None, corr_changed: bool = True) -> torch.Tensor:
@@ -648,11 +690,11 @@
             (self.fwd_band if inc else self.fwd)[name]()
         for name in ("conv5", "conv5_1", "conv6", "conv6_1"):
             self.fwd[name]()
-        self._pf_forward(6)
+        self._pf_forward(6, defer=True)
         for k in (5, 4, 3, 2):
             self._up_forward(k + 1)
             self.fwd[f"deconv{k}"]()
-            self._pf_forward(k)
+            self._pf_forward(k, defer=True)
         return self.flow[2]
 
     def backward(self, g_flow2: torch.Tensor, band=None, fused_window: bool = True, skip_unread: bool = True, tail_split: bool = True):
@@ -819,11 +861,11 @@
         stage("conv3_1", self.fwd["conv3_1"], lambda v: self.cat3.load_nchw(v, 0))
         for name in ("conv4", "conv4_1", "conv5", "conv5_1", "conv6", "conv6_1"):
             self.fwd[name]()
-        self._pf_forward(6)
+        self._pf_forward(6, defer=True)
         for k in (5, 4, 3, 2):
             self._up_forward(k + 1)
             self.fwd[f"deconv{k}"]()
-            self._pf_forward(k)
+            self._pf_forward(k, defer=True)
         return self.flow[2]
 
 
diff --git a/understanding_flow_robustness_amd/patch_attack.py b/understanding_flow_robustness_amd/patch_attack.py
--- a/understanding_flow_robustness_amd/patch_attack.py
+++ b/understanding_flow_robustness_amd/patch_attack.py
@@ -345,9 +345,9 @@
             flow = predict_flow(self.net, None, self.adv_tgt, self.adv_ref, self.args)
         weight = (1.0 - self.alpha) * ((1.0 / self.world) if self.shared else float(self.B))
         if flow is None:
-            L.check(L.lib().ufr_flow2_upsampled_loss(L.ptr(self.eng.flow_out), float(self.eng.flow_scale), L.ptr(self.target),
-                                                     L.ptr(self.g_flow2), L.ptr(self.loss_local), self.B, self.H // 4, self.W // 4,
-                                                     self.kind, weight, L.ptr(self.loss_ws), L.stream()), "upsampled flow loss")
+            L.check(L.lib().ufr_flow2_upsampled_loss_fast(L.ptr(self.eng.flow_out), float(self.eng.flow_scale), L.ptr(self.target),
+                                                          L.ptr(self.g_flow2), L.ptr(self.loss_local), self.B, self.H // 4, self.W // 4,
+                                                          self.kind, weight, L.ptr(self.loss_ws), L.stream()), "upsampled flow loss")
         else:
             if not flow.is_contiguous():
                 flow = flow.contiguous()
```
